# bharatlytics/faceRecognition_InfrenceEngine

Hardware: AMD Instinct MI355X
Metric: faces/sec end-to-end @1080p (higher is better)
Workload: dtype f16

## Files before the change

### facerecognition_infrenceengine_amd/_lib.py

```python
import ctypes as C
import struct
import os
import threading

_HERE = os.path.dirname(os.path.abspath(__file__))
LIB_PATH = os.path.join(_HERE, "csrc", "libfrhip.so")

_lock = threading.Lock()
_lib = None
ABI_VERSION = 106


class FrError(RuntimeError):
    pass


class ConvArgs(C.Structure):
    _fields_ = [("x", C.c_void_p), ("w", C.c_void_p), ("y", C.c_void_p),
                ("bias", C.c_void_p), ("slope", C.c_void_p), ("residual", C.c_void_p),
                ("out_f32_partial", C.c_void_p),
                ("B", C.c_int), ("H", C.c_int), ("W", C.c_int), ("Cin", C.c_int), ("Cout", C.c_int),
                ("KH", C.c_int), ("KW", C.c_int), ("stride", C.c_int), ("pad", C.c_int),
                ("Ho", C.c_int), ("Wo", C.c_int), ("bias_mode", C.c_int), ("splitk", C.c_int),
                ("x2", C.c_void_p), ("C2", C.c_int)]


class ConvStep(C.Structure):
    _fields_ = [("kind", C.c_int), ("args", ConvArgs)]


class ConvF8Args(C.Structure):
    _fields_ = [("x8", C.c_void_p), ("w8", C.c_void_p), ("y16", C.c_void_p), ("y8", C.c_void_p),
                ("oscale", C.c_void_p), ("bias", C.c_void_p), ("slope", C.c_void_p), ("residual", C.c_void_p),
                ("B", C.c_int), ("H", C.c_int), ("W", C.c_int), ("Cin", C.c_int), ("Cout", C.c_int),
                ("bias_mode", C.c_int), ("y8_mul", C.c_float), ("y8_sub", C.c_void_p)]


class RolePtr(C.c_void_p):
    role = None


class PnetLevel(C.Structure):
    _fields_ = [("x1", C.c_void_p), ("head", C.c_void_p), ("workspace", C.c_void_p), ("H1", C.c_int), ("W1", C.c_int),
                ("scale", C.c_float), ("boxes", C.c_void_p), ("scores", C.c_void_p), ("regs", C.c_void_p),
                ("counts", C.c_void_p), ("block_counts", C.c_void_p),
                ("x1s", C.c_void_p), ("hs", C.c_int), ("ws", C.c_int), ("f16", C.c_int)]


class FrameRef(C.Structure):
    _fields_ = [("data", C.c_void_p), ("H", C.c_int32), ("W", C.c_int32), ("nh", C.c_int32), ("nw", C.c_int32),
                ("reserved", C.c_int32 * 2)]


class Call(C.Structure):
    _fields_ = [("fn", C.c_int32), ("nargs", C.c_int32), ("a", C.c_uint64 * 22)]


_P, _I, _L, _F, _Z = C.c_void_p, C.c_int, C.c_int64, C.c_float, C.c_size_t
SEQ_FN = {"fr_dconv_mfma_f32": 1, "fr_pnet23_split_f16": 2, "fr_pnet_candidates": 3, "fr_sort_nms": 4, "fr_box_refine": 5,
          "fr_crop_conv1_f32": 6, "fr_stage_select": 7}

SIGNATURES = {
    "fr_version": (_I, []),
    "fr_last_error_string": (C.c_char_p, []),
    "fr_device_count": (_I, []),
    "fr_l2norm_rows_f32": (_I, [_P, _P, _I, _I, _P]),
    "fr_gallery_match_workspace": (_Z, [_I, _L]),
    "fr_gallery_match_f32": (_I, [_P, _P, _I, _L, _I, _L, _P, _P, _P, _Z, _P, _I, _P]),
    "fr_gallery_match_view_f32": (_I, [_P, _P, _P, _I, _L, _I, _P, _P, _P, _Z, _P]),
    "fr_gallery_topk_workspace": (_Z, [_I, _L, _I]),
    "fr_gallery_topk_f32": (_I, [_P, _P, _I, _L, _I, _I, _L, _P, _P, _P, _Z, _P, _I, _P]),
    "fr_gallery_topk_view_f32": (_I, [_P, _P, _P, _I, _L, _I, _I, _P, _P, _P, _Z, _P]),
    "fr_gallery_update_rows_f32": (_I, [_P, _P, _P, _I, _I, _I, _P]),
    "fr_gallery_match_f16_workspace": (_Z, [_I, _L]),
    "fr_gallery_match_f16": (_I, [_P, _P, _P, _I, _L, _I, _L, _P, _P, _P, _Z, _P, _I, _P]),
    "fr_gallery_match_f8_workspace": (_Z, [_I, _L]),
    "fr_gallery_match_f8": (_I, [_P, _P, _P, _I, _L, _I, _L, _P, _P, _P, _Z, _P, _I, _P]),
    "fr_gallery_update_rows_shadow": (_I, [_P, _P, _I, _P, _P, _I, _I, _I, _P]),
    "fr_gallery_match_view_f16_workspace": (_Z, [_I, _L]),
    "fr_gallery_match_view_f16": (_I, [_P, _P, _P, _P, _I, _L, _L, _I, _P, _P, _P, _Z, _P]),
    "fr_gallery_match_view_f8_workspace": (_Z, [_I, _L]),
    "fr_gallery_match_view_f8": (_I, [_P, _P, _P, _P, _I, _L, _L, _I, _P, _P, _P, _Z, _P]),
    "fr_gallery_topk_f16_workspace": (_Z, [_I, _L, _I]),
    "fr_gallery_topk_f16": (_I, [_P, _P, _P, _I, _L, _I, _I, _L, _P, _P, _P, _P, _P, _Z, _P, _I, _P]),
    "fr_gallery_topk_view_f16_workspace": (_Z, [_I, _L, _I]),
    "fr_gallery_topk_view_f16": (_I, [_P, _P, _P, _P, _I, _L, _L, _I, _I, _P, _P, _P, _P, _P, _Z, _P]),
    "fr_gallery_topk_view_masked_f32": (_I, [_P, _P, _P, _I, _L, _I, _I, _P, _P, _P, _Z, _P, _P]),
    "fr_gallery_match_grouped_workspace": (_Z, [_I, _L]),
    "fr_gallery_match_grouped_f32": (_I, [_P, _P, _P, _P, _P, _I, _I, _L, _L, _I, _P, _P, _P, _Z, _P, _I, _P]),
    "fr_gallery_topk_grouped_workspace": (_Z, [_I, _L, _I]),
    "fr_gallery_topk_grouped_f32": (_I, [_P, _P, _P, _P, _P, _I, _I, _L, _L, _I, _I, _P, _P, _P, _Z, _P, _I, _P]),
    "fr_gallery_gmax_update": (_I, [_P, _P, _L, _I, _P, _P]),
    "fr_f32_to_f8": (_I, [_P, _P, _L, _P]),
    "fr_f32_to_f16": (_I, [_P, _P, _L, _P]),
    "fr_match_decide": (_I, [_P, _P, _I, _F, _F, _P, _P]),
    "fr_match_pack_candidates": (_I, [_P, _P, _I, _P, _P]),
    "fr_match_reduce_shards": (_I, [_P, _I, _I, _I, _I, _P, _P, _P]),
    "fr_match_reduce_shards_topk": (_I, [_P, _I, _I, _I, _I, _I, _P, _P, _P]),
    "fr_exchange_pack_queries": (_I, [_P, _I, _I, _I, _P, _P]),
    "fr_exchange_counts": (_I, [_P, _I, _I, _I, _P, _P]),
    "fr_gallery_first_above_f32": (_I, [_P, _P, _I, _L, _I, _F, _I, _L, _P, _P, _P, _Z, _P]),
    "fr_cosine_matrix_f32": (_I, [_P, _P, _I, _I, _I, _P, _P]),
    "fr_mean_rows_f32": (_I, [_P, _I, _I, _P, _P]),
    "fr_unknown_assign_batch_f32": (_I, [_P, _P, _I, _I, _F, _P, _P, _P, _I, _I, _P, _P, _P, _P]),
    "fr_gallery_first_above_blocked_f32": (_I, [_P, _P, _P, _P, _I, _L, _I, _F, _I, _L, _P, _P, _P, _Z, _P]),
    "fr_enrol_batch_workspace": (_Z, [_I, _L]),
    "fr_enrol_batch_f32": (_I, [_P, _P, _I, _P, _P, _I, _P, _I, _I, _I, _P, _P, _L, _F, _F, _P, _P, _P, _P, _P, _P, _P, _P,
                                _Z, _P]),
    "fr_gallery_pairs_workspace": (_Z, [_L, _L]),
    "fr_gallery_pairs_above_f16": (_I, [_P, _P, _L, _I, _F, _I, _L, _I, _P, _P, _P, _P, _Z, _P]),
    "fr_conv_nhwc_f16": (_I, [C.POINTER(ConvArgs), _P]),
    "fr_conv_sequence": (_I, [C.POINTER(ConvStep), _I, _P]),
    "fr_conv_inblock_f16": (_I, [C.POINTER(ConvArgs), _P]),
    "fr_conv_nhwc_f8": (_I, [C.POINTER(ConvF8Args), _P]),
    "fr_quantize_f16_f8": (_I, [_P, _P, _L, _F, _P]),
    "fr_quantize_f16_f8_centred": (_I, [_P, _P, _L, _I, _P, _F, _P]),
    "fr_gptq_round_e4m3": (_I, [_P, _P, _P, _P, _I, _I, _P]),
    "fr_conv_stage14_weight_bytes": (_Z, [_I]),
    "fr_conv_stage14_pack": (_I, [_P, _P, _P]),
    "fr_conv_stage14_f16": (_I, [_P, _P, _P, _P, _I, _I, _P]),
    "fr_conv_walk64_weight_bytes": (_Z, [_I]),
    "fr_conv_walk64_pack": (_I, [_P, _P, _I, _P]),
    "fr_conv_walk64_f16": (_I, [_P, _P, _P, _P, _I, _P, _P, _I, _I, _I, _P]),
    "fr_conv_stage28_weight_bytes": (_Z, [_I]),
    "fr_conv_stage28_pack": (_I, [_P, _P, _P]),
    "fr_conv_stage28_f16": (_I, [_P, _P, _P, _P, _I, _I, _P]),
    "fr_conv_stage14_f8_weight_bytes": (_Z, [_I]),
    "fr_conv_stage14_f8_param_floats": (_Z, []),
    "fr_conv_stage14_f8_pack": (_I, [_P, _P, _P]),
    "fr_conv_stage14_f8": (_I, [_P, _P, _P, _P, _P, _I, _I, _P]),
    "fr_conv_splitk_epilogue": (_I, [_P, _I, _I, _I, _I, _I, _P, _I, _P, _P, _P, _P]),
    "fr_fc_reduce_l2norm": (_I, [_P, _I, _I, _I, _P, _P, _P, _P]),
    "fr_warp_affine_5pt": (_I, [_P, _I, _I, _I, _P, _P, _P, _I, _I, _P, _P, _P, _P]),
    "fr_warp_affine_5pt_slots": (_I, [_P, _I, _I, _I, _P, _P, _I, _I, _P, _P]),
    "fr_warp_affine_5pt_refs": (_I, [_P, _I, _P, _P, _P, _I, _I, _P, _P, _P, _P]),
    "fr_warp_affine_5pt_slots_refs": (_I, [_P, _I, _P, _P, _I, _I, _P, _P]),
    "fr_letterbox_u8": (_I, [_P, _I, _P, _I, _I, _P]),
    "fr_detections_unscale": (_I, [_P, _P, _P, _P, _I, _I, _P]),
    "fr_yuv420_to_bgr_u8": (_I, [_P, _P, _I, _I, _I, _I, _I, _I, _I, _I, _I, _I, _P]),
    "fr_yuv420_to_bgr_refs_u8": (_I, [_P, _P, _I, _I, _I, _I, _I, _I, _I, _I, _P]),
    "fr_frame_activity_u8": (_I, [_P, _I, _I, _I, _P, _I, _P, _P, _P, _I, _P, _P, _P, _I, _I, _I, _P]),
    "fr_frame_activity_refs_u8": (_I, [_P, _I, _P, _I, _P, _P, _P, _I, _P, _P, _P, _I, _I, _I, _P]),
    "fr_pyramid_resize_norm":(_I, [_P, _I, _I, _I, _I, _I, _P, _P]),
    "fr_dconv_f32": (_I, [_P, _P, _P, _P, _P, _I, _I, _I, _I, _I, _I, _I, _I, _I, _P, _P, _I, _P]),
    "fr_dconv_mfma_f32": (_I, [_I, _P, _P, _P, _P, _P, _I, _I, _I, _P, _P, _P, _I, _I, _P, _I, _P, _P]),
    "fr_crop_conv1_f32": (_I, [_I, _P, _I, _I, _I, _P, _P, _I, _P, _P, _P, _P, _P]),
    "fr_crop_conv1_split": (_I, [_I, _P, _I, _I, _I, _P, _P, _I, _P, _P, _P, _P, _I, _P]),
    "fr_crop_conv1_list_f32": (_I, [_I, _P, _I, _I, _I, _P, _I, _P, _P, _I, _P, _P, _P, _P, _P]),
    "fr_ro_conv2_split": (_I, [_I, _P, _P, _P, _P, _P, _I, _P, _I, _P, _P]),
    "fr_ro_gemm_weight_bytes": (_Z, [_I]),
    "fr_ro_gemm_pack": (_I, [_I, _P, _P, _P]),
    "fr_ro_gemm_split": (_I, [_I, _P, _P, _P, _P, _P, _I, _P, _I, _P]),
    "fr_ro_margin_list": (_I, [_P, _I, _P, _I, _I, _F, _F, _P, _P, _I, _P]),
    "fr_ro_scatter_rows": (_I, [_P, _P, _P, _I, _I, _P, _P]),
    "fr_pnet23_workspace_bytes": (_Z, [_I, _I, _I]),
    "fr_pnet23_split_f16": (_I, [_P, _P, _I, _I, _I, _P, _P, _P, _P, _P, _P, _P, _P, _P, _I, _F, _F, _P, _P, _Z, _P]),
    "fr_maxpool_f32": (_I, [_P, _P, _I, _I, _I, _I, _I, _I, _P]),
    "fr_pnet_conv1_band": (_I, [_I, _P, _I, _I, _I, _I, _I, _P, _P, _P, _P, _P, _P, _P, _I, _P]),
    "fr_pnet_band_tiles_count": (_Z, [_I, _I, _I]),
    "fr_pnet_band_tiles": (_I, [_P, _I, _I, _I, _P, _P, _P]),
    "fr_pnet_finish_levels": (_I, [C.POINTER(PnetLevel), _I, _I, _P, _P, _P, _P, _P, _P, _P, _P, _F, _I, _F, _P, _P]),
    "fr_pnet_pyramid_conv1": (_I, [_I, _P, _I, _I, _I, C.POINTER(PnetLevel), _I, _P, _P, _P, _P, _P, _I, _P]),
    "fr_pnet_pyramid_p23": (_I, [C.POINTER(PnetLevel), _I, _I, _P, _P, _P, _P, _P, _P, _P, _P, _I, _F, _F, _P]),
    "fr_pnet_pyramid_band_tiles": (_I, [C.POINTER(PnetLevel), _I, _I, _P, _P, _P]),
    "fr_pnet_candidates": (_I, [_P, _I, _I, _I, _F, _F, _I, _P, _P, _P, _P, _P, _P, _P, _F, _P]),
    "fr_sort_nms": (_I, [_P, _P, _P, _I, _P, _I, _I, _I, _I, _F, _I, _I, _P, _P, _P, _P, _I, _P]),
    "fr_box_refine": (_I, [_P, _P, _I, _P, _I, _I, _I, _P]),
    "fr_crop_resize_norm": (_I, [_P, _I, _I, _I, _P, _P, _I, _I, _P, _P]),
    "fr_stage_select": (_I, [_P, _P, _I, _P, _I, _I, _F, _P, _P, _P, _I, _P, _P, _P]),
    "fr_detect_sequence": (_I, [C.POINTER(Call), _I]),
    "fr_det_conv_weight_halves": (_Z, [_I, _I, _I]),
    "fr_det_conv_f16": (_I, [_P, _P, _P, _P, _P, _I, _I, _I, _I, _I, _I, _I, _I, _I, _I, _I, _I, _I, _I, _I, _P]),
    "fr_det_conv_act_f16": (_I, [_P, _P, _P, _P, _P, _P, _I, _I, _I, _I, _I, _I, _I, _I, _I, _I, _I, _I, _I, _I, _I, _P]),
    "fr_dw_conv_f16": (_I, [_P, _P, _P, _P, _P, _I, _I, _I, _I, _I, _I, _I, _I, _I, _I, _P]),
    "fr_det_input_f16": (_I, [_P, _P, _I, _I, _I, _P]),
    "fr_det_pool_f16": (_I, [_P, _P, _I, _I, _I, _I, _I, _I, _I, _I, _I, _I, _P]),
    "fr_det_upsample_add_f16": (_I, [_P, _P, _P, _I, _I, _I, _I, _I, _P]),
    "fr_scrfd_decode": (_I, [_P, _P, _P, _I, _I, _I, _I, _I, _I, _F, _P, _I, _P, _P, _P, _P, _P]),
}

_NOCHECK = ("fr_version", "fr_device_count")


def _slot(v, t):
    if t is _F:
        return struct.unpack("<I", struct.pack("<f", float(v)))[0]
    if t is _P:
        if v is None:
            return 0
        return int(v.value or 0) if isinstance(v, C.c_void_p) else int(v)
    return int(v) & 0xFFFFFFFFFFFFFFFF


class Lib:

    def __init__(self, cdll):
        self._c = cdll
        self._calls = {}
        self._rec = threading.local()
        for name, (res, args) in SIGNATURES.items():
            fn = getattr(cdll, name)
            fn.restype = res
            fn.argtypes = args
            if res is _I and name not in _NOCHECK:
                self._calls[name] = self._checked(name, fn)
            else:
                self._calls[name] = fn

    def _checked(self, name, fn):
        err = self._c.fr_last_error_string

        fid, types, rec = SEQ_FN.get(name), fn.argtypes, self._rec

        def call(*a):
            rc = fn(*a)
            if rc != 0:
                raise FrError(f"{name} failed ({rc}): {err().decode()}")
            if getattr(rec, "calls", None) is not None:
                rec.invalid = name
            return rc

        def call_rec(*a):
            rc = fn(*a)
            if rc != 0:
                raise FrError(f"{name} failed ({rc}): {err().decode()}")
            calls = getattr(rec, "calls", None)
            if calls is not None:
                calls.append((fid, [_slot(v, t) for v, t in zip(a, types)],
                              [(i, v.role) for i, v in enumerate(a) if isinstance(v, RolePtr)]))
            return rc
        return call_rec if fid is not None else call

    def start_recording(self):
        self._rec.calls, self._rec.invalid = [], None

    def note(self, fid, *slots):
        calls = getattr(self._rec, "calls", None)
        if calls is not None:
            calls.append((fid, [int(v.value or 0) if isinstance(v, C.c_void_p) else int(v) for v in slots], []))

    def stop_recording(self):
        calls, self._rec.calls = getattr(self._rec, "calls", None), None
        self._rec.last_invalid = getattr(self._rec, "invalid", None)
        self._rec.invalid = None
        return None if self._rec.last_invalid else calls

    def recording_invalid(self):
        return getattr(self._rec, "last_invalid", None)

    def __getattr__(self, name):
        try:
            return self.__dict__["_calls"][name]
        except KeyError:
            raise AttributeError(name)


def load():
    global _lib
    with _lock:
        if _lib is None:
            import torch
            if not os.path.exists(LIB_PATH):
                raise FrError(f"{LIB_PATH} not built: run `python -c 'import __graft_entry__ as g; g.build()'` "
                              f"or `make -C {os.path.dirname(LIB_PATH)}`; there is no CPU fallback")
            lib = Lib(C.CDLL(LIB_PATH))
            have = lib.fr_version()
            if have != ABI_VERSION:
                raise FrError(f"{LIB_PATH} implements ABI version {have}, this binding needs {ABI_VERSION}: rebuild it "
                              f"(`make -C {os.path.dirname(LIB_PATH)}`)")
            _lib = lib
        return _lib


def ptr(t, role=None):
    if t is None:
        return None
    if role is None:
        return C.c_void_p(t.data_ptr())
    p = RolePtr(t.data_ptr())
    p.role = role
    return p


def stream_ptr():
    import torch
    return C.c_void_p(torch.cuda.current_stream().cuda_stream)


def require_gpu():
    import torch
    if not torch.cuda.is_available():
        raise FrError("no HIP device visible: this engine has no CPU path")
```

### facerecognition_infrenceengine_amd/csrc/pnet_fused.hip

```cpp
#include "detect_math.h"

#define P23_RH 8
#define P23_RW 32
#define P23_X1W (P23_RW + 4)
#define P23_X1PX ((P23_RH + 4) * P23_X1W)
#define P23_X2W (P23_RW + 2)
#define P23_X2PX ((P23_RH + 2) * P23_X2W)
#define P23_X2T ((P23_X2PX + 15) / 16)
#define P23_NT 512
#define P23_X1PL (448 * 32)
#define P23_X2PL (P23_X2PX * 32)

struct P23Args {
    const float* x1;
    const unsigned char* x1s;
    unsigned x1s_bytes;
    const float* w2; const float* b2; const float* s2;
    const float* w3; const float* b3; const float* s3;
    const float* hw; const float* hb;
    float* head;
    float* dl;
    int all_heads;
    int* list; int* counts; int seg_cap;
    float logit_thr;
    float band_hi;
    int B, H1, W1, H3, W3, tiles_x, tiles_y, ntiles;
};

__device__ __forceinline__ void pnet23_body(const P23Args& a, const int vb, const int vgrid, char* lds) {
#if defined(__HIP_DEVICE_COMPILE__)
    char* x1t = lds;
    char* x2t = x1t + 2 * P23_X1PL;
    char* wf = x2t + 2 * P23_X2PL;
    float* cst = reinterpret_cast<float*>(wf + 30 * 1024);
    int* lcnt = reinterpret_cast<int*>(cst + 104);
    const int tid = threadIdx.x, lane = tid & 63, wave = tid >> 6;
    const int fr = lane & 15, fq = lane >> 4;

    for (int e = tid; e < 30 * 64; e += P23_NT) {
        const int l2 = e & 63, plane = (e >> 6) & 1, slot = e >> 7;
        const int r = l2 & 15, q = l2 >> 4;
        const bool c3 = slot >= 5;
        const int ct = c3 ? (slot - 5) / 5 : 0, ks = c3 ? (slot - 5) % 5 : slot;
        const float* w = (c3 ? a.w3 : a.w2) + ((size_t)(ct * 16 + r) * 10 + 2 * ks + (q >> 1)) * 16 + 8 * (q & 1);
        half8 o;
#pragma unroll
        for (int j = 0; j < 8; ++j) o[j] = split_f16_plane(w[j], plane);
        *reinterpret_cast<half8*>(wf + (size_t)e * 16) = o;
    }
    for (int e = tid; e < 16; e += P23_NT) { cst[e] = a.b2[e]; cst[16 + e] = a.s2[e] - 1.f; }
    for (int e = tid; e < 32; e += P23_NT) { cst[32 + e] = a.b3[e]; cst[64 + e] = a.s3[e] - 1.f; }
    for (int e = tid; e < 8; e += P23_NT) cst[96 + e] = e < 6 ? a.hb[e] : 0.f;
    if (tid == 0) *lcnt = 0;
    int* const seg = a.list + (size_t)vb * a.seg_cap;

    int off2[5], off3[5];
#pragma unroll
    for (int ks = 0; ks < 5; ++ks) {
        int t = 2 * ks + (fq >> 1);
        if (t > 8) t = 8;
        off2[ks] = ((t / 3) * P23_X1W + t % 3) * 32 + (fq & 1) * 16;
        off3[ks] = ((t / 3) * P23_X2W + t % 3) * 32 + (fq & 1) * 16;
    }

    __amdgpu_buffer_rsrc_t xrs = buffer_rsrc(a.x1s, a.x1s_bytes);
    int wy[4], wx[4], wc[4];
#pragma unroll
    for (int i = 0; i < 4; ++i) {
        const int j = wave + 8 * i, pl = j >= 14 ? 1 : 0;
        const int p = (j - 14 * pl) * 32 + (lane >> 1);
        wy[i] = p < P23_X1PX ? p / P23_X1W : 1 << 20; wx[i] = p % P23_X1W;
        wc[i] = pl * 32 + (lane & 1) * 16;
    }
    auto issue_window = [&](int tile) {
        const int per = a.tiles_x * a.tiles_y;
        const int n = tile / per, rem = tile - n * per;
        const int ty0 = (rem / a.tiles_x) * P23_RH, tx0 = (rem % a.tiles_x) * P23_RW;
#pragma unroll
        for (int i = 0; i < 4; ++i) {
            const int j = wave + 8 * i;
            if (j < 28) {
                const int gy = ty0 + wy[i], gx = tx0 + wx[i];
                const unsigned off = (gy < a.H1 && gx < a.W1) ? (unsigned)(((n * a.H1 + gy) * a.W1 + gx) * 64 + wc[i]) : 0x80000000u;
                __builtin_amdgcn_raw_ptr_buffer_load_lds(xrs, (lds_ptr_t)(x1t + (j >= 14 ? P23_X1PL + (j - 14) * 1024 : j * 1024)), 16, off, 0, 0, 0);
            }
        }
    };

    __syncthreads();
    half8 hwh, hwl;
#pragma unroll
    for (int j = 0; j < 8; ++j) {
        const int co = j < 4 ? 4 * fq + j : 16 + 4 * fq + (j - 4);
        const float w = fr < 6 ? a.hw[co * 6 + fr] : 0.f;
        split_f16(w, hwh, hwl, j);
    }
    issue_window(vb);
    for (int tile = vb; tile < a.ntiles; tile += vgrid) {
        const int per = a.tiles_x * a.tiles_y;
        const int n = tile / per, rem = tile - n * per;
        const int ty0 = (rem / a.tiles_x) * P23_RH, tx0 = (rem % a.tiles_x) * P23_RW;
        asm volatile("s_waitcnt vmcnt(0)" ::: "memory");
        __syncthreads();
        {
            const int t0 = wave < 6 ? wave * 3 : 18 + (wave - 6) * 2, nt = wave < 6 ? 3 : 2;
            int pb[3];
            float4v acc[3];
#pragma unroll
            for (int t = 0; t < 3; ++t) {
                int q = (t0 + t) * 16 + fr;
                if (q >= P23_X2PX) q = 0;
                pb[t] = ((q / P23_X2W) * P23_X1W + q % P23_X2W) * 32;
                acc[t] = float4v{0.f, 0.f, 0.f, 0.f};
            }
#pragma unroll
            for (int ks = 0; ks < 5; ++ks) {
                const half8 ahi = *reinterpret_cast<const half8*>(wf + ((ks * 2 + 0) * 64 + lane) * 16);
                const half8 alo = *reinterpret_cast<const half8*>(wf + ((ks * 2 + 1) * 64 + lane) * 16);
#pragma unroll
                for (int t = 0; t < 3; ++t) {
                    if (t < nt) {
                        const char* bp = x1t + (pb[t] + off2[ks]);
                        const half8 bhi = *reinterpret_cast<const half8*>(bp);
                        const half8 blo = *reinterpret_cast<const half8*>(bp + P23_X1PL);
                        acc[t] = __builtin_amdgcn_mfma_f32_16x16x32_f16(alo, bhi, acc[t], 0, 0, 0);
                        acc[t] = __builtin_amdgcn_mfma_f32_16x16x32_f16(ahi, blo, acc[t], 0, 0, 0);
                        acc[t] = __builtin_amdgcn_mfma_f32_16x16x32_f16(ahi, bhi, acc[t], 0, 0, 0);
                    }
                }
            }
            const float4v bb = *reinterpret_cast<const float4v*>(cst + 4 * fq), ss = *reinterpret_cast<const float4v*>(cst + 16 + 4 * fq);
#pragma unroll
            for (int t = 0; t < 3; ++t) {
                const int q = (t0 + t) * 16 + fr;
                if (t < nt && q < P23_X2PX) {
                    float4v v = acc[t] + bb;
#pragma unroll
                    for (int e = 0; e < 4; ++e) v[e] = __builtin_fmaf(fminf(v[e], 0.f), ss[e], v[e]);
                    half4 hi, lo;
#pragma unroll
                    for (int e = 0; e < 4; ++e) split_f16(v[e], hi, lo, e);
                    char* o = x2t + q * 32 + fq * 8;
                    *reinterpret_cast<half4*>(o) = hi;
                    *reinterpret_cast<half4*>(o + P23_X2PL) = lo;
                }
            }
        }
        __syncthreads();
        if (tile + vgrid < a.ntiles) issue_window(tile + vgrid);
        {
            int pb[2];
            float4v acc[2][2];
#pragma unroll
            for (int t = 0; t < 2; ++t) {
                const int q = (wave * 2 + t) * 16 + fr;
                pb[t] = ((q >> 5) * P23_X2W + (q & 31)) * 32;
                acc[t][0] = acc[t][1] = float4v{0.f, 0.f, 0.f, 0.f};
            }
#pragma unroll
            for (int ks = 0; ks < 5; ++ks) {
                half8 ahi[2], alo[2];
#pragma unroll
                for (int ct = 0; ct < 2; ++ct) {
                    ahi[ct] = *reinterpret_cast<const half8*>(wf + (((5 + ct * 5 + ks) * 2 + 0) * 64 + lane) * 16);
                    alo[ct] = *reinterpret_cast<const half8*>(wf + (((5 + ct * 5 + ks) * 2 + 1) * 64 + lane) * 16);
                }
#pragma unroll
                for (int t = 0; t < 2; ++t) {
                    const char* bp = x2t + (pb[t] + off3[ks]);
                    const half8 bhi = *reinterpret_cast<const half8*>(bp);
                    const half8 blo = *reinterpret_cast<const half8*>(bp + P23_X2PL);
#pragma unroll
                    for (int ct = 0; ct < 2; ++ct) {
                        acc[t][ct] = __builtin_amdgcn_mfma_f32_16x16x32_f16(alo[ct], bhi, acc[t][ct], 0, 0, 0);
                        acc[t][ct] = __builtin_amdgcn_mfma_f32_16x16x32_f16(ahi[ct], blo, acc[t][ct], 0, 0, 0);
                        acc[t][ct] = __builtin_amdgcn_mfma_f32_16x16x32_f16(ahi[ct], bhi, acc[t][ct], 0, 0, 0);
                    }
                }
            }
            const float4v b30 = *reinterpret_cast<const float4v*>(cst + 32 + 4 * fq), s30 = *reinterpret_cast<const float4v*>(cst + 64 + 4 * fq);
            const float4v b31 = *reinterpret_cast<const float4v*>(cst + 48 + 4 * fq), s31 = *reinterpret_cast<const float4v*>(cst + 80 + 4 * fq);
#pragma unroll
            for (int t = 0; t < 2; ++t) {
                float4v v0 = acc[t][0] + b30, v1 = acc[t][1] + b31;
                half8 bh, bl;
#pragma unroll
                for (int e = 0; e < 4; ++e) {
                    const float x0 = __builtin_fmaf(fminf(v0[e], 0.f), s30[e], v0[e]), x1 = __builtin_fmaf(fminf(v1[e], 0.f), s31[e], v1[e]);
                    const half_t h0 = (half_t)x0, h1 = (half_t)x1;
                    bh[e] = h0; bl[e] = (half_t)(x0 - (float)h0);
                    bh[4 + e] = h1; bl[4 + e] = (half_t)(x1 - (float)h1);
                }
                float4v d = {0.f, 0.f, 0.f, 0.f};
                d = __builtin_amdgcn_mfma_f32_16x16x32_f16(hwl, bh, d, 0, 0, 0);
                d = __builtin_amdgcn_mfma_f32_16x16x32_f16(hwh, bl, d, 0, 0, 0);
                d = __builtin_amdgcn_mfma_f32_16x16x32_f16(hwh, bh, d, 0, 0, 0);
                const int q = (wave * 2 + t) * 16 + fr;
                const int gy = ty0 + (q >> 5), gx = tx0 + (q & 31);
                const bool inb = fq < 2 && gy < a.H3 && gx < a.W3;
                const size_t cell = ((size_t)n * a.H3 + gy) * a.W3 + gx;
                const float4v hb4 = *reinterpret_cast<const float4v*>(cst + 96 + 4 * (fq & 1));
                const float o0 = d[0] + hb4[0], o1 = d[1] + hb4[1];
                const float dlv = __shfl(o1 - o0, fr, 64);
                const bool band = a.band_hi > a.logit_thr;
                const bool flag = inb && fq == 0 && (split_nonfinite(dlv) || (dlv >= a.logit_thr && (!band || dlv <= a.band_hi)));
                const unsigned long long fm = __ballot(flag);
                if (fm) {
                    int base = 0;
                    if (lane == (int)__builtin_ctzll(fm)) base = atomicAdd(lcnt, (int)__builtin_popcountll(fm));
                    base = __shfl(base, (int)__builtin_ctzll(fm), 64);
                    if (flag) seg[base + (int)__builtin_popcountll(fm & ((1ull << lane) - 1ull))] = (int)cell;
                }
                if (inb) {
                    if (fq == 0) a.dl[cell] = o1 - o0;
                    if (a.all_heads || (band && dlv >= a.logit_thr)) {
                        float* o = a.head + cell * 6 + 4 * fq;
                        *reinterpret_cast<float2*>(o) = make_float2(o0, o1);
                        if (fq == 0) *reinterpret_cast<float2*>(o + 2) = make_float2(d[2] + hb4[2], d[3] + hb4[3]);
                    }
                }
            }
        }
    }
    __syncthreads();
    if (tid == 0) a.counts[vb] = *lcnt;
#endif
}

__global__ __launch_bounds__(P23_NT, 4) void pnet23_split_f16(P23Args a) {
    extern __shared__ __attribute__((aligned(16))) char lds[];
    pnet23_body(a, (int)blockIdx.x, (int)gridDim.x, lds);
}

#define P23_MAXL 16
struct P23Levels {
    const unsigned char* x1s[P23_MAXL]; float* head[P23_MAXL]; float* dl[P23_MAXL];
    int H1[P23_MAXL], W1[P23_MAXL], seg_cap[P23_MAXL], first[P23_MAXL + 1];
    int nlevels;
};
__global__ __launch_bounds__(P23_NT, 4) void pnet23_split_levels(P23Args a, P23Levels t) {
    extern __shared__ __attribute__((aligned(16))) char lds[];
    int l = 0;
    while (l + 1 < t.nlevels && (int)blockIdx.x >= t.first[l + 1]) ++l;
    a.H1 = t.H1[l]; a.W1 = t.W1[l]; a.H3 = a.H1 - 4; a.W3 = a.W1 - 4;
    a.tiles_x = (a.W3 + P23_RW - 1) / P23_RW; a.tiles_y = (a.H3 + P23_RH - 1) / P23_RH;
    a.ntiles = a.B * a.tiles_x * a.tiles_y;
    a.x1s = t.x1s[l]; a.x1s_bytes = (unsigned)a.B * a.H1 * a.W1 * 64; a.head = t.head[l];
    a.dl = t.dl[l]; a.counts = reinterpret_cast<int*>(a.dl + (size_t)a.B * a.H3 * a.W3); a.list = a.counts + 512;
    a.seg_cap = t.seg_cap[l];
    pnet23_body(a, (int)blockIdx.x - t.first[l], t.first[l + 1] - t.first[l], lds);
}

#define PREF_WS 304
struct PRefArgs {
    const float* x1; const float* w2; const float* b2; const float* s2; const float* w3; const float* b3; const float* s3;
    const float* hw; const float* hb; float* head;
    const int* list; const int* counts; int seg_cap;
    int B, H1, W1, H3, W3;
    int* counter;
};

__device__ __forceinline__ void pnet_refine_body(const PRefArgs& a, const int block, float (*wins)[16 * PREF_WS], int (*cbase)[16]) {
#if defined(__HIP_DEVICE_COMPILE__)
    const int tid = threadIdx.x, lane = tid & 63, wave = tid >> 6;
    const int li = lane & 15, kq = lane >> 4;
    float* win = wins[wave];
    if (a.counts[block] <= wave * 16) return;
    float wa2[27], wa3[2][36], hwa[8];
#pragma unroll
    for (int s = 0; s < 27; ++s) wa2[s] = a.w2[(li * 10 + s / 3) * 16 + 4 * (s % 3) + kq];
#pragma unroll
    for (int i = 0; i < 2; ++i)
#pragma unroll
        for (int s = 0; s < 36; ++s) wa3[i][s] = a.w3[((16 * i + li) * 10 + s / 4) * 16 + 4 * (s % 4) + kq];
#pragma unroll
    for (int i = 0; i < 2; ++i)
#pragma unroll
        for (int e = 0; e < 4; ++e) hwa[i * 4 + e] = li < 6 ? a.hw[(16 * i + 4 * kq + e) * 6 + li] : 0.f;
    const float4v b2 = *reinterpret_cast<const float4v*>(a.b2 + 4 * kq), s2 = *reinterpret_cast<const float4v*>(a.s2 + 4 * kq);
    float4v b3[2], s3[2], hb4;
#pragma unroll
    for (int i = 0; i < 2; ++i) {
        b3[i] = *reinterpret_cast<const float4v*>(a.b3 + 16 * i + 4 * kq);
        s3[i] = *reinterpret_cast<const float4v*>(a.s3 + 16 * i + 4 * kq);
    }
#pragma unroll
    for (int r = 0; r < 4; ++r) hb4[r] = kq * 4 + r < 6 ? a.hb[kq * 4 + r] : 0.f;

    const int hw3 = a.H3 * a.W3;
    {
        const int* lst = a.list + (size_t)block * a.seg_cap;
        const int n_list = a.counts[block];
        if (a.counter && tid == 0 && n_list) atomicAdd(a.counter, n_list);
        for (int i0 = wave * 16; i0 < n_list; i0 += 64) {
            {
                const int c = lst[min(i0 + li, n_list - 1)];
                const int n = c / hw3, r = c - n * hw3, y = r / a.W3, x = r - y * a.W3;
                if (kq == 0) cbase[wave][li] = ((n * a.H1 + y) * a.W1 + x) * 12;
            }
            __builtin_amdgcn_wave_barrier();
            int l_ = lane;
            asm volatile("" : "+v"(l_));
            float4v pf[19];
#pragma unroll
            for (int it = 0; it < 19; ++it) {
                const int idx = min(it * 64 + l_, 1199);
                const int j = idx / 75, rem = idx - j * 75, row = rem / 15, c4 = rem - row * 15;
                pf[it] = *reinterpret_cast<const float4v*>(a.x1 + (size_t)(unsigned)cbase[wave][j] + (row * a.W1 * 12 + c4 * 4));
            }
#pragma unroll
            for (int it = 0; it < 19; ++it) {
                const int idx = it * 64 + l_;
                const int j = idx / 75, rem = idx - j * 75, row = rem / 15, c4 = rem - row * 15;
                if (it < 18 || l_ < 48) *reinterpret_cast<float4v*>(win + j * PREF_WS + row * 60 + c4 * 4) = pf[it];
            }
            __builtin_amdgcn_wave_barrier();
            const float* xb = win + li * PREF_WS + kq;
            float4v acc2[9];
#pragma unroll
            for (int p = 0; p < 9; ++p) acc2[p] = float4v{0.f, 0.f, 0.f, 0.f};
#pragma unroll
            for (int s = 0; s < 27; ++s) {
                const int tap = s / 3, c4 = s - tap * 3, ty = tap / 3, tx = tap - ty * 3;
#pragma unroll
                for (int p = 0; p < 9; ++p) {
                    const int py = p / 3, px = p - py * 3;
                    acc2[p] = __builtin_amdgcn_mfma_f32_16x16x4f32(wa2[s], xb[((py + ty) * 5 + px + tx) * 12 + 4 * c4], acc2[p], 0, 0, 0);
                }
            }
            __builtin_amdgcn_wave_barrier();
#pragma unroll
            for (int p = 0; p < 9; ++p) {
                float4v v = acc2[p] + b2;
#pragma unroll
                for (int e = 0; e < 4; ++e) v[e] = v[e] > 0.f ? v[e] : v[e] * s2[e];
                *reinterpret_cast<float4v*>(win + li * PREF_WS + p * 16 + 4 * kq) = v;
            }
            __builtin_amdgcn_wave_barrier();
            float4v acc3[2] = {float4v{0.f, 0.f, 0.f, 0.f}, float4v{0.f, 0.f, 0.f, 0.f}};
#pragma unroll
            for (int s = 0; s < 36; ++s) {
                const float bv = xb[(s / 4) * 16 + 4 * (s % 4)];
#pragma unroll
                for (int i = 0; i < 2; ++i) acc3[i] = __builtin_amdgcn_mfma_f32_16x16x4f32(wa3[i][s], bv, acc3[i], 0, 0, 0);
            }
            float4v hd = hb4;
#pragma unroll
            for (int i = 0; i < 2; ++i) {
                float4v v = acc3[i] + b3[i];
#pragma unroll
                for (int e = 0; e < 4; ++e) v[e] = v[e] > 0.f ? v[e] : v[e] * s3[i][e];
#pragma unroll
                for (int e = 0; e < 4; ++e) hd = __builtin_amdgcn_mfma_f32_16x16x4f32(hwa[i * 4 + e], v[e], hd, 0, 0, 0);
            }
            if (i0 + li < n_list && kq < 2) {
                float* o = a.head + (size_t)lst[i0 + li] * 6 + 4 * kq;
                *reinterpret_cast<float2*>(o) = make_float2(hd[0], hd[1]);
                if (kq == 0) *reinterpret_cast<float2*>(o + 2) = make_float2(hd[2], hd[3]);
            }
            __builtin_amdgcn_wave_barrier();
        }
    }
#endif
}

__global__ __launch_bounds__(256, 2) void pnet_refine_mfma(PRefArgs a) {
    __shared__ __attribute__((aligned(16))) float wins[4][16 * PREF_WS];
    __shared__ int cbase[4][16];
    pnet_refine_body(a, blockIdx.x, wins, cbase);
}

#define PREF_MAXL 16
struct PRefLevels {
    const float* x1[PREF_MAXL]; float* head[PREF_MAXL]; const int* list[PREF_MAXL]; const int* counts[PREF_MAXL];
    int seg_cap[PREF_MAXL], H1[PREF_MAXL], W1[PREF_MAXL], first[PREF_MAXL + 1];
    int nlevels;
};
__global__ __launch_bounds__(256, 2) void pnet_refine_levels(PRefArgs a, PRefLevels t) {
    __shared__ __attribute__((aligned(16))) float wins[4][16 * PREF_WS];
    __shared__ int cbase[4][16];
    int l = 0;
    while (l + 1 < t.nlevels && (int)blockIdx.x >= t.first[l + 1]) ++l;
    a.x1 = t.x1[l]; a.head = t.head[l]; a.list = t.list[l]; a.counts = t.counts[l]; a.seg_cap = t.seg_cap[l];
    a.H1 = t.H1[l]; a.W1 = t.W1[l]; a.H3 = t.H1[l] - 4; a.W3 = t.W1[l] - 4;
    pnet_refine_body(a, (int)blockIdx.x - t.first[l], wins, cbase);
}

static void p23_layout(int B, int H1, int W1, long long& ncell, long long& ntiles, int& grid, int& seg_cap) {
    const int H3 = H1 - 4, W3 = W1 - 4;
    ncell = (long long)B * H3 * W3;
    ntiles = (long long)B * ((W3 + P23_RW - 1) / P23_RW) * ((H3 + P23_RH - 1) / P23_RH);
    grid = (int)(ntiles < 512 ? ntiles : 512);
    seg_cap = (int)((ntiles + grid - 1) / (grid > 0 ? grid : 1)) * (P23_RH * P23_RW);
}
extern "C" size_t fr_pnet23_workspace_bytes(int B, int H1, int W1) {
    if (B <= 0 || H1 < 5 || W1 < 5) return 0;
    long long ncell, ntiles; int grid, seg_cap;
    p23_layout(B, H1, W1, ncell, ntiles, grid, seg_cap);
    return (size_t)ncell * 4 + 512 * 4 + (size_t)grid * seg_cap * 4;
}

extern "C" int fr_pnet23_split_f16(const float* x1, const void* x1s, int B, int H1, int W1, const float* w2, const float* b2,
                                   const float* s2, const float* w3, const float* b3, const float* s3, const float* hw,
                                   const float* hb, float* head, int all_heads, float refine_logit_thr, float refine_band_hi,
                                   int32_t* refined_count, void* workspace, size_t workspace_bytes, fr_stream_t stream) {
    FR_REQUIRE(x1 && x1s && w2 && b2 && s2 && w3 && b3 && s3 && hw && hb && head, "fr_pnet23_split_f16: null pointer");
    FR_REQUIRE((int64_t)B * H1 * W1 * 64 < (1ll << 31), "fr_pnet23_split_f16: the split conv1 map must stay below 2 GiB (got %lld bytes)", (long long)B * H1 * W1 * 64);
    FR_REQUIRE(B > 0 && H1 >= 5 && W1 >= 5, "fr_pnet23_split_f16: the conv1 map must be at least 5x5 (got %dx%d)", H1, W1);
    P23Args a;
    a.x1 = x1; a.x1s = (const unsigned char*)x1s; a.x1s_bytes = (unsigned)((int64_t)B * H1 * W1 * 64); a.w2 = w2; a.b2 = b2; a.s2 = s2; a.w3 = w3; a.b3 = b3; a.s3 = s3; a.hw = hw; a.hb = hb; a.head = head; a.all_heads = all_heads & 1;
    a.B = B; a.H1 = H1; a.W1 = W1; a.H3 = H1 - 4; a.W3 = W1 - 4;
    a.tiles_x = (a.W3 + P23_RW - 1) / P23_RW; a.tiles_y = (a.H3 + P23_RH - 1) / P23_RH;
    long long ncell, nt; int grid, seg_cap;
    p23_layout(B, H1, W1, ncell, nt, grid, seg_cap);
    FR_REQUIRE(nt < (1ll << 31) && ncell < (1ll << 31), "fr_pnet23_split_f16: too many tiles");
    const size_t need = fr_pnet23_workspace_bytes(B, H1, W1);
    FR_REQUIRE(workspace && workspace_bytes >= need, "fr_pnet23_split_f16: workspace needs %zu bytes (fr_pnet23_workspace_bytes)", need);
    a.dl = reinterpret_cast<float*>(workspace);
    a.counts = reinterpret_cast<int*>(a.dl + ncell);
    a.list = a.counts + 512;
    a.seg_cap = seg_cap;
    a.logit_thr = refine_logit_thr;
    a.band_hi = refine_band_hi;
    a.ntiles = (int)nt;
    constexpr size_t lds = (size_t)2 * P23_X1PL + (size_t)2 * P23_X2PL + 30 * 1024 + 108 * 4;
    static FrDevLatch latch;
    if (!fr_raise_lds(reinterpret_cast<const void*>(pnet23_split_f16), lds, latch)) { fr_set_error("fr_pnet23_split_f16: cannot raise dynamic LDS"); return FR_E_LAUNCH; }
    hipStream_t s = fr_stream(stream);
    pnet23_split_f16<<<grid, P23_NT, lds, s>>>(a);
    FR_CHECK_LAUNCH("pnet23_split_f16");
    if (all_heads & 2) return FR_OK;
    PRefArgs r;
    r.x1 = x1; r.w2 = w2; r.b2 = b2; r.s2 = s2; r.w3 = w3; r.b3 = b3; r.s3 = s3; r.hw = hw; r.hb = hb; r.head = head;
    r.list = a.list; r.counts = a.counts; r.seg_cap = seg_cap;
    r.B = B; r.H1 = H1; r.W1 = W1; r.H3 = a.H3; r.W3 = a.W3; r.counter = refined_count;
    pnet_refine_mfma<<<grid, 256, 0, s>>>(r);
    FR_CHECK_LAUNCH("pnet_refine_mfma");
    return FR_OK;
}

int fr_pnet_candidates_levels_launch(const fr_pnet_level* lv, int nlevels, int nframes, float thr, int cap, float dl_min, hipStream_t s);

extern "C" int fr_pnet_finish_levels(const fr_pnet_level* levels, int nlevels, int nframes, const float* w2, const float* b2,
                                     const float* s2, const float* w3, const float* b3, const float* s3, const float* hw,
                                     const float* hb, float thr, int cap, float dl_min, int32_t* refined_count, fr_stream_t stream) {
    FR_REQUIRE(levels && nlevels > 0 && nlevels <= PREF_MAXL && nframes > 0 && cap > 0, "fr_pnet_finish_levels: 1 .. %d levels", PREF_MAXL);
    FR_REQUIRE(w2 && b2 && s2 && w3 && b3 && s3 && hw && hb, "fr_pnet_finish_levels: null pointer");
    PRefLevels t;
    t.nlevels = nlevels;
    int total = 0;
    for (int l = 0; l < nlevels; ++l) {
        const fr_pnet_level& L = levels[l];
        FR_REQUIRE(L.x1 && L.head && L.workspace && L.boxes && L.scores && L.regs && L.counts && L.block_counts && L.H1 >= 5 && L.W1 >= 5 && L.scale > 0.f,
                   "fr_pnet_finish_levels: level %d: bad entry", l);
        long long ncell, nt; int grid, seg_cap;
        p23_layout(nframes, L.H1, L.W1, ncell, nt, grid, seg_cap);
        float* dl = reinterpret_cast<float*>(L.workspace);
        const int* counts = reinterpret_cast<const int*>(dl + ncell);
        t.x1[l] = L.x1; t.head[l] = L.head; t.counts[l] = counts; t.list[l] = counts + 512;
        t.seg_cap[l] = seg_cap; t.H1[l] = L.H1; t.W1[l] = L.W1;
        t.first[l] = total;
        total += grid;
    }
    t.first[nlevels] = total;
    PRefArgs r;
    r.x1 = nullptr; r.w2 = w2; r.b2 = b2; r.s2 = s2; r.w3 = w3; r.b3 = b3; r.s3 = s3; r.hw = hw; r.hb = hb; r.head = nullptr;
    r.list = nullptr; r.counts = nullptr; r.seg_cap = 0; r.B = nframes; r.H1 = r.W1 = r.H3 = r.W3 = 0; r.counter = refined_count;
    hipStream_t s = fr_stream(stream);
    pnet_refine_levels<<<total, 256, 0, s>>>(r, t);
    FR_CHECK_LAUNCH("pnet_refine_levels");
    return fr_pnet_candidates_levels_launch(levels, nlevels, nframes, thr, cap, dl_min, s);
}

__global__ __launch_bounds__(256) void pnet_band_tiles_kernel(const int* __restrict__ list, const int* __restrict__ counts, int seg_cap,
                                                             int H3, int W3, int regions_x, int regions_y, int32_t* __restrict__ tbuf,
                                                             int32_t* __restrict__ tiles) {
    const int n_list = counts[blockIdx.x];
    const int* lst = list + (size_t)blockIdx.x * seg_cap;
    const int hw3 = H3 * W3;
    for (int i = threadIdx.x; i < n_list; i += 256) {
        const int c = lst[i];
        const int n = c / hw3, r = c - n * hw3, y = r / W3, x = r - y * W3;
        const int ry0 = (2 * y) >> 4, ry1 = min((2 * y + 9) >> 4, regions_y - 1);
        const int rx0 = (2 * x) >> 6, rx1 = min((2 * x + 9) >> 6, regions_x - 1);
        for (int ry = ry0; ry <= ry1; ++ry)
            for (int rx = rx0; rx <= rx1; ++rx) {
                const int t = (n * regions_y + ry) * regions_x + rx;
                const unsigned bit = 1u << (t & 31);
                const unsigned old = atomicOr(reinterpret_cast<unsigned*>(tbuf) + 1 + (t >> 5), bit);
                if (!(old & bit)) tiles[atomicAdd(tbuf, 1)] = t;
            }
    }
}

extern "C" size_t fr_pnet_band_tiles_count(int B, int H1, int W1) {
    if (B <= 0 || H1 < 5 || W1 < 5) return 0;
    return (size_t)B * ((H1 + 7) / 8) * ((W1 + 31) / 32);
}

extern "C" int fr_pnet_band_tiles(const void* workspace, int B, int H1, int W1, int32_t* tbuf, int32_t* tiles, fr_stream_t stream) {
    FR_REQUIRE(workspace && tbuf && tiles && B > 0 && H1 >= 5 && W1 >= 5, "fr_pnet_band_tiles: bad argument");
    long long ncell, nt; int grid, seg_cap;
    p23_layout(B, H1, W1, ncell, nt, grid, seg_cap);
    const float* dl = reinterpret_cast<const float*>(workspace);
    const int* counts = reinterpret_cast<const int*>(dl + ncell);
    const int regions_y = (H1 + 7) / 8, regions_x = (W1 + 31) / 32;
    const size_t ntile = (size_t)B * regions_y * regions_x;
    hipStream_t s = fr_stream(stream);
    if (hipMemsetAsync(tbuf, 0, (1 + (ntile + 31) / 32) * sizeof(int32_t), s) != hipSuccess) { fr_set_error("fr_pnet_band_tiles: memset failed"); return FR_E_LAUNCH; }
    pnet_band_tiles_kernel<<<grid, 256, 0, s>>>(counts + 512, counts, seg_cap, H1 - 4, W1 - 4, regions_x, regions_y, tbuf, tiles);
    FR_CHECK_LAUNCH("pnet_band_tiles_kernel");
    return FR_OK;
}

extern "C" int fr_pnet_pyramid_p23(const fr_pnet_level* levels, int nlevels, int nframes, const float* w2, const float* b2,
                                   const float* s2, const float* w3, const float* b3, const float* s3, const float* hw,
                                   const float* hb, int all_heads, float refine_logit_thr, float refine_band_hi, fr_stream_t stream) {
    FR_REQUIRE(levels && nlevels > 0 && nlevels <= P23_MAXL && nframes > 0, "fr_pnet_pyramid_p23: 1 .. %d levels", P23_MAXL);
    FR_REQUIRE(w2 && b2 && s2 && w3 && b3 && s3 && hw && hb, "fr_pnet_pyramid_p23: null pointer");
    P23Levels t;
    t.nlevels = nlevels;
    long long total = 0;
    for (int l = 0; l < nlevels; ++l) {
        const fr_pnet_level& L = levels[l];
        FR_REQUIRE(L.x1s && L.head && L.workspace && L.H1 >= 5 && L.W1 >= 5, "fr_pnet_pyramid_p23: level %d: bad entry", l);
        FR_REQUIRE((int64_t)nframes * L.H1 * L.W1 * 64 < (1ll << 31), "fr_pnet_pyramid_p23: level %d: the split conv1 map must stay below 2 GiB", l);
        long long ncell, nt; int grid, seg_cap;
        p23_layout(nframes, L.H1, L.W1, ncell, nt, grid, seg_cap);
        t.x1s[l] = reinterpret_cast<const unsigned char*>(L.x1s); t.head[l] = L.head; t.dl[l] = reinterpret_cast<float*>(L.workspace);
        t.H1[l] = L.H1; t.W1[l] = L.W1; t.seg_cap[l] = seg_cap;
        t.first[l] = (int)total;
        total += grid;
    }
    t.first[nlevels] = (int)total;
    P23Args a{};
    a.w2 = w2; a.b2 = b2; a.s2 = s2; a.w3 = w3; a.b3 = b3; a.s3 = s3; a.hw = hw; a.hb = hb; a.all_heads = all_heads & 1;
    a.logit_thr = refine_logit_thr; a.band_hi = refine_band_hi; a.B = nframes;
    constexpr size_t lds = (size_t)2 * P23_X1PL + (size_t)2 * P23_X2PL + 30 * 1024 + 108 * 4;
    static FrDevLatch latch;
    if (!fr_raise_lds(reinterpret_cast<const void*>(pnet23_split_levels), lds, latch)) { fr_set_error("fr_pnet_pyramid_p23: cannot raise dynamic LDS"); return FR_E_LAUNCH; }
    pnet23_split_levels<<<(unsigned)total, P23_NT, lds, fr_stream(stream)>>>(a, t);
    FR_CHECK_LAUNCH("pnet23_split_levels");
    return FR_OK;
}

struct PBandLevels {
    const int* counts[PREF_MAXL];
    int seg_cap[PREF_MAXL], H1[PREF_MAXL], W1[PREF_MAXL], word0[PREF_MAXL], level[PREF_MAXL], first[PREF_MAXL + 1];
    int nlevels;
};
__global__ __launch_bounds__(256) void pnet_band_tiles_levels(PBandLevels t, int32_t* __restrict__ tbuf, int32_t* __restrict__ tiles, int cap) {
    int l = 0;
    while (l + 1 < t.nlevels && (int)blockIdx.x >= t.first[l + 1]) ++l;
    const int b = (int)blockIdx.x - t.first[l];
    const int n_list = t.counts[l][b];
    const int* lst = t.counts[l] + 512 + (size_t)b * t.seg_cap[l];
    const int H3 = t.H1[l] - 4, W3 = t.W1[l] - 4, hw3 = H3 * W3;
    const int regions_y = (t.H1[l] + 7) / 8, regions_x = (t.W1[l] + 31) / 32;
    unsigned* bitmap = reinterpret_cast<unsigned*>(tbuf) + 1 + t.word0[l];
    for (int i = threadIdx.x; i < n_list; i += 256) {
        const int c = lst[i];
        const int n = c / hw3, r = c - n * hw3, y = r / W3, x = r - y * W3;
        const int ry0 = (2 * y) >> 4, ry1 = min((2 * y + 9) >> 4, regions_y - 1);
        const int rx0 = (2 * x) >> 6, rx1 = min((2 * x + 9) >> 6, regions_x - 1);
        for (int ry = ry0; ry <= ry1; ++ry)
            for (int rx = rx0; rx <= rx1; ++rx) {
                const int tl = (n * regions_y + ry) * regions_x + rx;
                const unsigned bit = 1u << (tl & 31);
                const unsigned old = atomicOr(bitmap + (tl >> 5), bit);
                if (!(old & bit)) {
                    const int at = atomicAdd(tbuf, 1);
                    if (at < cap) tiles[at] = (t.level[l] << 27) | tl;
                }
            }
    }
}

extern "C" int fr_pnet_pyramid_band_tiles(const fr_pnet_level* levels, int nlevels, int nframes, int32_t* tbuf, int32_t* tiles,
                                          fr_stream_t stream) {
    FR_REQUIRE(levels && nlevels > 0 && nlevels <= PREF_MAXL && nframes > 0 && tbuf && tiles, "fr_pnet_pyramid_band_tiles: bad argument");
    PBandLevels t;
    t.nlevels = 0;
    long long blocks = 0, words = 0, cap = 0;
    for (int l = 0; l < nlevels; ++l) {
        const fr_pnet_level& L = levels[l];
        if (!L.f16) continue;
        FR_REQUIRE(L.workspace && L.H1 >= 5 && L.W1 >= 5, "fr_pnet_pyramid_band_tiles: level %d: bad entry", l);
        long long ncell, nt; int grid, seg_cap;
        p23_layout(nframes, L.H1, L.W1, ncell, nt, grid, seg_cap);
        const long long ntile = (long long)fr_pnet_band_tiles_count(nframes, L.H1, L.W1);
        FR_REQUIRE(ntile < (1ll << 27), "fr_pnet_pyramid_band_tiles: level %d: too many tiles", l);
        const int k = t.nlevels++;
        t.counts[k] = reinterpret_cast<const int*>(reinterpret_cast<const float*>(L.workspace) + ncell);
        t.seg_cap[k] = seg_cap; t.H1[k] = L.H1; t.W1[k] = L.W1; t.word0[k] = (int)words; t.level[k] = l;
        t.first[k] = (int)blocks;
        blocks += grid; words += (ntile + 31) / 32; cap += ntile;
    }
    FR_REQUIRE(t.nlevels > 0 && cap < (1ll << 31), "fr_pnet_pyramid_band_tiles: no level in the f16 form");
    t.first[t.nlevels] = (int)blocks;
    hipStream_t s = fr_stream(stream);
    if (hipMemsetAsync(tbuf, 0, (size_t)(1 + words) * sizeof(int32_t), s) != hipSuccess) { fr_set_error("fr_pnet_pyramid_band_tiles: memset failed"); return FR_E_LAUNCH; }
    pnet_band_tiles_levels<<<(unsigned)blocks, 256, 0, s>>>(t, tbuf, tiles, (int)cap);
    FR_CHECK_LAUNCH("pnet_band_tiles_levels");
    return FR_OK;
}
```

### facerecognition_infrenceengine_amd/mtcnn.py

```python
import contextlib
import ctypes
import functools
import logging
import math
import threading
from types import SimpleNamespace
from typing import NamedTuple

import torch

from . import _lib


def pyramid_scales(h, w, minsize=20, factor=0.709):
    m = 12.0 / minsize
    minl = min(h, w) * m
    scales, k = [], 0
    while minl >= 12:
        scales.append(m * factor ** k)
        minl *= factor
        k += 1
    return scales


def _pool_out(n, k, s):
    o = -(-(n - k) // s) + 1
    if (o - 1) * s >= n:
        o -= 1
    return o


MFMA_LAYERS = {0: (3, 12, 3, 3, 1), 1: (12, 16, 3, 3, 1), 2: (16, 32, 3, 3, 2),
               10: (4, 28, 3, 3, 2), 11: (28, 48, 3, 3, 3), 12: (48, 64, 2, 2, 4), 13: (64, 128, 3, 3, 4),
               14: (128, 6, 1, 1, 1),
               20: (4, 32, 3, 3, 1), 21: (32, 64, 3, 3, 2), 22: (64, 64, 3, 3, 4), 23: (64, 128, 2, 2, 4),
               24: (128, 256, 3, 3, 4), 25: (256, 16, 1, 1, 1)}


class _MConv:

    def __init__(self, layer, w, b, slope, device, head=None):
        cin, cout, kh, kw, ntb = MFMA_LAYERS[layer]
        rcout, rcin = w.shape[0], w.shape[1]
        assert tuple(w.shape[2:]) == (kh, kw) and rcout <= cout and rcin <= cin, (layer, tuple(w.shape))
        wfull = torch.zeros((cout, cin, kh, kw), dtype=torch.float32)
        wfull[:rcout, :rcin] = w
        w = wfull
        bfull = torch.zeros(cout); bfull[:rcout] = b; b = bfull
        if slope is not None:
            sfull = torch.zeros(cout); sfull[:rcout] = slope; slope = sfull
        self.layer, self.cin, self.cout, self.kh, self.kw = layer, cin, cout, kh, kw
        cinp = -(-cin // 4) * 4
        cp = ntb * 16 + (16 if ntb % 2 == 0 else 0)
        gsz = ntb * 16
        ngroups = -(-cout // gsz)
        wp = torch.zeros((ngroups, kh * kw, cinp, cp), dtype=torch.float32)
        wt = w.permute(2, 3, 1, 0).reshape(kh * kw, cin, cout)
        for g in range(ngroups):
            n = min(gsz, cout - g * gsz)
            wp[g, :, :cin, :n] = wt[:, :, g * gsz:g * gsz + n]
        self.w = wp.contiguous().to(device)
        bp = torch.zeros(ngroups * gsz); bp[:cout] = b
        self.b = bp.to(device)
        self.slope = None
        if slope is not None:
            sp = torch.zeros(ngroups * gsz); sp[:cout] = slope
            self.slope = sp.to(device)
        self.head_w = self.head_b = None
        self.nhead = 0
        if head is not None:
            self.head_w = head[0].t().contiguous().to(torch.float32).to(device)
            self.head_b = head[1].to(torch.float32).contiguous().to(device)
            self.nhead = head[0].shape[0]
        self.pool = {0: 2, 10: 3, 11: 3, 20: 3, 21: 3, 22: 2}.get(layer, 0)

    def out_hw(self, h, w):
        hc, wc = h - self.kh + 1, w - self.kw + 1
        return (_pool_out(hc, self.pool, 2), _pool_out(wc, self.pool, 2)) if self.pool else (hc, wc)


_CHAINS = {"pnet": (("conv1", ("conv2",)), ("conv2", ("conv3",)), ("conv3", ("conv4_1", "conv4_2"))),
           "rnet": (("conv1", ("conv2",)), ("conv2", ("conv3",)), ("conv3", ("dense4",)), ("dense4", ("dense5_1", "dense5_2"))),
           "onet": (("conv1", ("conv2",)), ("conv2", ("conv3",)), ("conv3", ("conv4",)), ("conv4", ("dense5",)),
                    ("dense5", ("dense6_1", "dense6_2", "dense6_3")))}


def canonical_scale(state, net, dead_zone=2):
    st = dict(state)
    for name, readers in _CHAINS[net]:
        w = st[name + ".weight"]
        rms = float(w.double().pow(2).mean().sqrt())
        if rms == 0.0:
            continue
        e = math.log2(math.sqrt(2.0 / w[0].numel()) / rms)
        k = int(round(e)) if abs(e) > dead_zone else 0
        if k:
            st[name + ".weight"] = w * 2.0 ** k
            st[name + ".bias"] = st[name + ".bias"] * 2.0 ** k
            for n in readers:
                st[n + ".weight"] = st[n + ".weight"] * 2.0 ** -k
    return st


def _dense_as_conv(w, k, c):
    o = w.shape[0]
    return w.reshape(o, k, k, c).permute(0, 3, 2, 1).contiguous()


class DetectSettings:
    SINGLE_FRAME_LEVEL_STREAMS = 4
    one_stream = False
    level_streams = 2
    phase_marks = None
    solo_max_frames = 7
    pnet_band = True
    split_pconv1 = True
    split_pconv1_min_px = 10000
    pyramid_launch = True
    refined_cells = None
    use_sequence = True
    fused_crop = True
    split_ro = True

    def __init__(self, minsize=20, factor=0.709, fused_pnet=True, batch_min_pixels=None):
        self.minsize, self.factor = minsize, factor
        self.fused_pnet = bool(fused_pnet)
        self.batch_min_pixels = 22_000_000 if batch_min_pixels is None else int(batch_min_pixels)
        self.single_frame_level_streams = self.SINGLE_FRAME_LEVEL_STREAMS


class DetectPlan(NamedTuple):
    N: int
    scales: tuple
    geo: tuple
    batch: bool
    few: bool
    band: bool
    fused: tuple
    f16: tuple
    pyramid: bool
    solo: bool
    nside: int
    cache: bool
    recorder: bool
    split: bool
    chunks: tuple


def _is_batch(cfg, N, H, W):
    return N * H * W >= cfg.batch_min_pixels


def _level_geo(H, W, scale):
    hs, ws = int(math.ceil(H * scale)), int(math.ceil(W * scale))
    return hs, ws, _pool_out(hs - 2, 2, 2), _pool_out(ws - 2, 2, 2)


def _frames32(h, w):
    return (2 ** 31 - 1) // (h * w * 64)


def _f16_conv1(cfg, band, h, w):
    return bool(band and cfg.split_pconv1 and h * w >= cfg.split_pconv1_min_px)


def detect_plan(N, H, W, cfg, trace=False, level_streams=None, out=False, capturing=False):
    return _plan(N, H, W, tuple([getattr(cfg, k) for k in _PLAN_READS]), cfg.phase_marks is None and cfg.refined_cells is None,
                 trace, level_streams, out, capturing)


_PLAN_READS = ("minsize", "factor", "fused_pnet", "batch_min_pixels", "solo_max_frames", "pnet_band", "split_pconv1", "split_pconv1_min_px",
               "pyramid_launch", "one_stream", "level_streams", "single_frame_level_streams", "split_ro", "fused_crop", "use_sequence")


@functools.lru_cache(maxsize=256)
def _plan(N, H, W, settings, recordable, trace, level_streams, out, capturing):
    cfg = SimpleNamespace(**dict(zip(_PLAN_READS, settings)))
    scales = tuple(pyramid_scales(H, W, cfg.minsize, cfg.factor))
    geo = tuple(_level_geo(H, W, s) for s in scales)
    batch = _is_batch(cfg, N, H, W)
    few = N <= cfg.solo_max_frames and not batch
    fusable = bool(cfg.fused_pnet) and not trace
    chunks, per = (), N
    if fusable and not out and N > 1 and geo and 1 <= _frames32(*geo[0][2:]) < N:
        per = -(-N // -(-N // _frames32(*geo[0][2:])))
        chunks = tuple((n0, min(N, n0 + per)) for n0 in range(0, N, per))
    band = bool(cfg.pnet_band and batch and not trace)
    fused = tuple(bool(cfg.fused_pnet) and per <= _frames32(h, w) for _, _, h, w in geo)
    f16 = tuple(fu and _f16_conv1(cfg, band, h, w) for fu, (_, _, h, w) in zip(fused, geo))
    pyramid = bool(cfg.pyramid_launch and batch and fusable and all(fused))
    nside = max(1, min(2, level_streams if level_streams is not None else cfg.level_streams))
    own = few and level_streams is None
    if own and capturing and cfg.single_frame_level_streams > 0:
        nside = min(cfg.single_frame_level_streams, max(1, len(scales) - 1))
    eager = bool(trace or cfg.one_stream or (own and not capturing))
    cache = bool(eager and few and not trace and not out and not capturing)
    recorder = bool(cache and recordable and cfg.use_sequence and cfg.fused_pnet and cfg.fused_crop and not cfg.one_stream)
    split = bool(cfg.split_ro and cfg.fused_crop and batch and not trace)
    return DetectPlan(N, scales, geo, batch, few, band, fused, f16, pyramid, eager or pyramid, nside, cache, recorder, split, chunks)


_RO = (SimpleNamespace(name="rnet", cap_in="cap_p", cap_out="cap_r", crop=24, map1=(11, 28), map2=(4, 48), w1="_rc1", w2="_rc2",
                       layers=("r1", "r2", "r3", "r4", "r5"), nhead=6, naux=4, refine=1),
       SimpleNamespace(name="onet", cap_in="cap_r", cap_out="cap_o", crop=48, map1=(23, 32), map2=(10, 64), w1="_oc1", w2="_oc2",
                       layers=("o1", "o2", "o3", "o4", "o5", "o6"), nhead=16, naux=14, refine=2))


class MTCNNHIP(DetectSettings):
    def __init__(self, pstate, rstate, ostate, device="cuda:0", minsize=20, factor=0.709,
                 thresholds=(0.6, 0.7, 0.7), cap_scale=2048, keep_scale=256, cap_p=512, cap_r=64, cap_o=16,
                 fused_pnet=True, batch_min_pixels=None, canonical=True):
        _lib.require_gpu()
        DetectSettings.__init__(self, minsize, factor, fused_pnet, batch_min_pixels)
        self.lib = _lib.load()
        self.device = torch.device(device)
        self.thresholds = tuple(float(t) for t in thresholds)
        self.cap_scale, self.keep_scale, self.cap_p, self.cap_r, self.cap_o = cap_scale, keep_scale, cap_p, cap_r, cap_o
        assert cap_scale <= 4096 and cap_p <= 1024 and cap_r <= 1024 and cap_o <= 1024
        self._sides = {}
        self._tls = threading.local()
        self._unfused_logged = False
        d = self.device
        p, r, o = ({k: v.detach().float().cpu() for k, v in s.items()} for s in (pstate, rstate, ostate))
        if canonical:
            p, r, o = (canonical_scale(s, n) for s, n in ((p, "pnet"), (r, "rnet"), (o, "onet")))
        self.p1 = _MConv(0, p["conv1.weight"], p["conv1.bias"], p["prelu1.weight"], d)
        self.p2 = _MConv(1, p["conv2.weight"], p["conv2.bias"], p["prelu2.weight"], d)
        hw = torch.cat([p["conv4_1.weight"].reshape(2, 32), p["conv4_2.weight"].reshape(4, 32)])
        hb = torch.cat([p["conv4_1.bias"], p["conv4_2.bias"]])
        self.p3 = _MConv(2, p["conv3.weight"], p["conv3.bias"], p["prelu3.weight"], d, head=(hw, hb))
        w2p = torch.zeros((16, 10, 16)); w2p[:, :9, :10] = p["conv2.weight"].permute(0, 2, 3, 1).reshape(16, 9, 10)
        w3p = torch.zeros((32, 10, 16)); w3p[:, :9, :16] = p["conv3.weight"].permute(0, 2, 3, 1).reshape(32, 9, 16)
        self._p23 = tuple(t.to(torch.float32).contiguous().to(d) for t in (
            w2p, p["conv2.bias"], p["prelu2.weight"], w3p, p["conv3.bias"], p["prelu3.weight"], hw.t().contiguous(), hb))
        self.refine_margin = 2e-3
        self.level_tensors = None
        self.p23_all_heads = False
        self._rc1 = tuple(t.to(torch.float32).contiguous().to(d) for t in (
            r["conv1.weight"].permute(2, 3, 1, 0).reshape(27, 28), r["conv1.bias"], r["prelu1.weight"]))
        self._oc1 = tuple(t.to(torch.float32).contiguous().to(d) for t in (
            o["conv1.weight"].permute(2, 3, 1, 0).reshape(27, 32), o["conv1.bias"], o["prelu1.weight"]))
        self.split_conv1 = True
        self.ro_margin = 1e-3
        self.ro_list_cap = (1024, 256)
        def c2w(w):
            o, c = w.shape[0], w.shape[1]
            wp = torch.zeros((o, 9, 32))
            wp[:, :, :c] = w.permute(0, 2, 3, 1).reshape(o, 9, c)
            return wp
        self._rc2 = tuple(t.to(torch.float32).contiguous().to(d) for t in (c2w(r["conv2.weight"]), r["conv2.bias"], r["prelu2.weight"]))
        self._oc2 = tuple(t.to(torch.float32).contiguous().to(d) for t in (c2w(o["conv2.weight"]), o["conv2.bias"], o["prelu2.weight"]))
        self.r1 = _MConv(10, r["conv1.weight"], r["conv1.bias"], r["prelu1.weight"], d)
        self.r2 = _MConv(11, r["conv2.weight"], r["conv2.bias"], r["prelu2.weight"], d)
        self.r3 = _MConv(12, r["conv3.weight"], r["conv3.bias"], r["prelu3.weight"], d)
        self.r4 = _MConv(13, _dense_as_conv(r["dense4.weight"], 3, 64), r["dense4.bias"], r["prelu4.weight"], d)
        self.r5 = _MConv(14, torch.cat([r["dense5_1.weight"], r["dense5_2.weight"]]).reshape(6, 128, 1, 1),
                         torch.cat([r["dense5_1.bias"], r["dense5_2.bias"]]), None, d)
        self.o1 = _MConv(20, o["conv1.weight"], o["conv1.bias"], o["prelu1.weight"], d)
        self.o2 = _MConv(21, o["conv2.weight"], o["conv2.bias"], o["prelu2.weight"], d)
        self.o3 = _MConv(22, o["conv3.weight"], o["conv3.bias"], o["prelu3.weight"], d)
        self.o4 = _MConv(23, o["conv4.weight"], o["conv4.bias"], o["prelu4.weight"], d)
        self.o5 = _MConv(24, _dense_as_conv(o["dense5.weight"], 3, 128), o["dense5.bias"], o["prelu5.weight"], d)
        self._gemm = {}
        for lid, wconv, b, sl in ((12, r["conv3.weight"], r["conv3.bias"], r["prelu3.weight"]),
                                  (13, _dense_as_conv(r["dense4.weight"], 3, 64), r["dense4.bias"], r["prelu4.weight"]),
                                  (22, o["conv3.weight"], o["conv3.bias"], o["prelu3.weight"]),
                                  (23, o["conv4.weight"], o["conv4.bias"], o["prelu4.weight"]),
                                  (24, _dense_as_conv(o["dense5.weight"], 3, 128), o["dense5.bias"], o["prelu5.weight"])):
            wk = wconv.permute(0, 2, 3, 1).reshape(wconv.shape[0], -1).to(torch.float32).contiguous().to(d)
            packed = torch.empty(self.lib.fr_ro_gemm_weight_bytes(lid), dtype=torch.uint8, device=d)
            with torch.cuda.device(d):
                self.lib.fr_ro_gemm_pack(lid, _lib.ptr(wk), _lib.ptr(packed), _lib.stream_ptr())
                torch.cuda.synchronize(d)
            self._gemm[lid] = (packed, b.to(torch.float32).contiguous().to(d), sl.to(torch.float32).contiguous().to(d))
        self.o6 = _MConv(25, torch.cat([o["dense6_1.weight"], o["dense6_2.weight"], o["dense6_3.weight"]]).reshape(16, 256, 1, 1),
                         torch.cat([o["dense6_1.bias"], o["dense6_2.bias"], o["dense6_3.bias"]]), None, d)

    def set_exact(self, on=True):
        self.pnet_band = self.split_ro = not on
        return self

    @property
    def _dl(self):
        return getattr(self._tls, "dl", (None, 0.0))

    @property
    def _s(self):
        return self._tls.s

    @_s.setter
    def _s(self, v):
        self._tls.s = v

    def _new(self, shape, dtype):
        c = getattr(self._tls, "cache", None)
        if c is None:
            return torch.empty(shape, dtype=dtype, device=self.device)
        lst, i = c
        c[1] = i + 1
        if i < len(lst) and lst[i].shape == tuple(shape) and lst[i].dtype == dtype:
            return lst[i]
        t = torch.empty(shape, dtype=dtype, device=self.device)
        self._tls.cache_grew = True
        if i < len(lst):
            lst[i] = t
        else:
            lst.append(t)
        return t

    def _f32(self, *shape):
        return self._new(shape, torch.float32)

    def _i32(self, *shape):
        return self._new(shape, torch.int32)

    def _fptr(self, frames):
        return _lib.ptr(frames, role="frame")

    def _dconv(self, x, c, B, H, W, frames=None, counts=None, cap=0, y_split=None, y=None):
        ho, wo = c.out_hw(H, W)
        if y is None:
            y = self._f32(B, ho, wo, c.nhead if c.nhead else c.cout)
        fh, fw = (frames.shape[1], frames.shape[2]) if frames is not None else (0, 0)
        self.lib.fr_dconv_mfma_f32(c.layer, _lib.ptr(x), _lib.ptr(c.w), _lib.ptr(c.b), _lib.ptr(c.slope), _lib.ptr(y),
                                   B, H, W, _lib.ptr(c.head_w), _lib.ptr(c.head_b), self._fptr(frames), fh, fw,
                                   _lib.ptr(counts), cap, _lib.ptr(y_split), self._s)
        return y, ho, wo

    def _gemm_split(self, lid, x, B, shape, counts, cap):
        w, b, sl = self._gemm[lid]
        y = self._f32(B, *shape)
        self.lib.fr_ro_gemm_split(lid, _lib.ptr(x), _lib.ptr(w), _lib.ptr(b), _lib.ptr(sl), _lib.ptr(y), B, _lib.ptr(counts), cap, self._s)
        return y

    def _nms(self, boxes, scores, aux, naux, counts, L, nseg, seg_cap, seg_major, thr, mode, keep, out=None, results=False):
        if out is None:
            bo, so, co = self._f32(L, keep, 4), self._f32(L, keep), self._i32(L)
            ao = self._f32(L, keep, max(naux, 1))
        else:
            bo, so, ao, co = out
        po = [_lib.ptr(t, role="out%d" % i if results else None) for i, t in enumerate((bo, so, ao, co))]
        self.lib.fr_sort_nms(_lib.ptr(boxes), _lib.ptr(scores), _lib.ptr(aux), naux, _lib.ptr(counts), L, nseg, seg_cap,
                             seg_major, thr, mode, keep, *po, keep, self._s)
        return bo, so, ao, co

    def _band_logits(self, band=True):
        lt = math.log(self.thresholds[0] / (1.0 - self.thresholds[0]))
        return lt - self.refine_margin, lt + self.refine_margin if band else float("-inf")

    def _level_buffers(self, N, scale, geo, band, f16, cand):
        hs, ws, h, w = geo
        path = getattr(self._tls, "path", None)
        if path is not None:
            path["fused_levels"] += 1
            path["band_levels"] += int(band)
            if f16:
                path["pconv1_mfma_levels"].append((h, w))
        xs = self._new((N, h, w, 64), torch.uint8)
        x = self._f32(N, h, w, 12)
        head = self._f32(N, h - 4, w - 4, 6)
        wsp = self._new((self.lib.fr_pnet23_workspace_bytes(N, h, w) // 4,), torch.float32)
        bc = self._i32(N * (-(-(h - 4) * (w - 4) // 256)))
        entry = None
        if cand is not None:
            entry = _lib.PnetLevel(x.data_ptr(), head.data_ptr(), wsp.data_ptr(), h, w, float(scale), *[t.data_ptr() for t in cand],
                                   bc.data_ptr(), xs.data_ptr(), hs, ws, int(f16))
        return dict(h=h, w=w, f16=f16, x=x, xs=xs, head=head, wsp=wsp, bc=bc), entry

    def _level(self, frames, scale, geo, fused, band, f16, trace, cand):
        N, H, W, _ = frames.shape
        hs, ws, h, w = geo
        lib, p1 = self.lib, self.p1
        if not fused:
            if self.fused_pnet and not self._unfused_logged:
                self._unfused_logged = True
                logging.getLogger(__name__).warning("MTCNNHIP: a %d x %d pyramid level of %d frame(s) exceeds the fused P-Net's 32-bit map "
                                                    "offsets; it runs layer by layer (f32)", hs, ws, N)
            if getattr(self._tls, "path", None) is not None:
                self._tls.path["unfused_levels"] += 1
            x, h, w = self._dconv(None, p1, N, hs, ws, frames=frames)
            x, h, w = self._dconv(x, self.p2, N, h, w)
            head, h, w = self._dconv(x, self.p3, N, h, w)
            return head, h, w, self._i32(N * (-(-h * w // 256))), None, 0.0, None
        lo, hi = self._band_logits(band)
        t, entry = self._level_buffers(N, scale, geo, band, f16, cand[3:] if f16 else None)
        x, xs, head, wsp = t["x"], t["xs"], t["head"], t["wsp"]
        p1w, p23 = (_lib.ptr(p1.w), _lib.ptr(p1.b), _lib.ptr(p1.slope)), [_lib.ptr(v) for v in self._p23]
        if f16:
            lib.fr_pnet_conv1_band(0, self._fptr(frames), N, H, W, hs, ws, *p1w, None, _lib.ptr(xs), None, None, 0, self._s)
        else:
            self._dconv(None, p1, N, hs, ws, frames=frames, y_split=xs, y=x)
        lib.fr_pnet23_split_f16(_lib.ptr(x), _lib.ptr(xs), N, h, w, *p23, _lib.ptr(head),
                                (1 if (self.p23_all_heads or trace is not None) else 0) | (2 if f16 else 0), lo, hi,
                                _lib.ptr(self.refined_cells), _lib.ptr(wsp), wsp.numel() * 4, self._s)
        keep = None
        if f16:
            nt = lib.fr_pnet_band_tiles_count(N, h, w)
            tbuf, tiles = self._i32(1 + (nt + 31) // 32), self._i32(nt)
            lib.fr_pnet_band_tiles(_lib.ptr(wsp), N, h, w, _lib.ptr(tbuf), _lib.ptr(tiles), self._s)
            lib.fr_pnet_conv1_band(1, self._fptr(frames), N, H, W, hs, ws, *p1w, _lib.ptr(x), None, _lib.ptr(tiles), _lib.ptr(tbuf), nt, self._s)
            lib.fr_pnet_finish_levels((_lib.PnetLevel * 1)(entry), 1, N, *p23, cand[1], cand[2], lo, _lib.ptr(self.refined_cells), self._s)
            t.update(tbuf=tbuf, tiles=tiles)
            keep = (x, xs, head, wsp, tbuf, tiles, t["bc"])
        if self.level_tensors is not None:
            self.level_tensors.append(t)
        return head, h - 4, w - 4, t["bc"], wsp, lo, keep

    def pnet_level(self, frames, scale, trace=None, cand=None):
        N, H, W, _ = frames.shape
        geo = _level_geo(H, W, scale)
        fused = bool(self.fused_pnet) and N <= _frames32(*geo[2:])
        band = bool(self.pnet_band and _is_batch(self, N, H, W) and trace is None)
        f16 = fused and cand is not None and _f16_conv1(self, band, *geo[2:])
        head, hc, wc, _, dl, dl_min, keep = self._level(frames, scale, geo, fused, band, f16, trace, cand)
        self._tls.dl, self._tls.level_done, self._tls.keep = (dl, dl_min), keep is not None, keep
        return head, hc, wc

    def _pnet_pyramid(self, frames, plan, cand):
        N, H, W, _ = frames.shape
        lib, p1, nlev = self.lib, self.p1, len(plan.scales)
        lo, hi = self._band_logits(plan.band)
        lv = (_lib.PnetLevel * nlev)()
        keep, ntile, words = [], 0, 0
        for li, (s, geo, f16) in enumerate(zip(plan.scales, plan.geo, plan.f16)):
            t, lv[li] = self._level_buffers(N, s, geo, plan.band, f16, [c[li] for c in cand])
            keep.append(t)
            if f16:
                nt = lib.fr_pnet_band_tiles_count(N, t["h"], t["w"])
                ntile, words = ntile + nt, words + (nt + 31) // 32
        p1w, p23 = (_lib.ptr(p1.w), _lib.ptr(p1.b), _lib.ptr(p1.slope)), [_lib.ptr(t) for t in self._p23]
        lib.fr_pnet_pyramid_conv1(0, self._fptr(frames), N, H, W, lv, nlev, *p1w, None, None, 0, self._s)
        lib.fr_pnet_pyramid_p23(lv, nlev, N, *p23, 1 if self.p23_all_heads else 0, lo, hi, self._s)
        if ntile:
            tbuf, tiles = self._i32(1 + words), self._i32(ntile)
            lib.fr_pnet_pyramid_band_tiles(lv, nlev, N, _lib.ptr(tbuf), _lib.ptr(tiles), self._s)
            lib.fr_pnet_pyramid_conv1(1, self._fptr(frames), N, H, W, lv, nlev, *p1w, _lib.ptr(tiles), _lib.ptr(tbuf), ntile, self._s)
            keep[0].update(tbuf=tbuf, tiles=tiles)
        lib.fr_pnet_finish_levels(lv, nlev, N, *p23, self.thresholds[0], self.cap_scale, lo, _lib.ptr(self.refined_cells), self._s)
        if self.level_tensors is not None:
            self.level_tensors.extend(keep)

    @contextlib.contextmanager
    def _forked(self, main, n, events=None):
        note = self.lib.note
        sides = self._sides.setdefault(main.cuda_stream, [])
        while len(sides) < n:
            sides.append(torch.cuda.Stream(device=self.device))
        sides = sides[:n]
        if events is None:
            for side in sides:
                side.wait_stream(main)
        else:
            events[0].record(main)
            note(8, events[0].cuda_event, main.cuda_stream)
            for side in sides:
                side.wait_event(events[0])
                note(9, side.cuda_stream, events[0].cuda_event)
        yield sides
        if events is None:
            for side in sides:
                main.wait_stream(side)
        else:
            for side, ev in zip(sides, events[1:]):
                ev.record(side)
                note(8, ev.cuda_event, side.cuda_stream)
                main.wait_event(ev)
                note(9, main.cuda_stream, ev.cuda_event)
        self._s = ctypes.c_void_p(main.cuda_stream)

    def _pnet_levels(self, frames, plan, trace, cand):
        N, lib, t0, cs = plan.N, self.lib, self.thresholds[0], self.cap_scale
        events = (self._tls.rec or {}).get("events")
        forked = events is not None or not plan.solo
        main, keep = torch.cuda.current_stream(), []
        with (self._forked(main, len(events) - 1 if events else plan.nside, events) if forked else contextlib.nullcontext()) as sides:
            for li, s in enumerate(plan.scales):
                stream = sides[(li - 1) % len(sides)] if forked and li else main
                with (contextlib.nullcontext() if plan.solo else torch.cuda.stream(stream)):
                    if forked:
                        self._s = ctypes.c_void_p(stream.cuda_stream)
                    lcand = [c[li] for c in cand]
                    head, hc, wc, bc, dl, dl_min, done = self._level(
                        frames, s, plan.geo[li], plan.fused[li], plan.band, plan.f16[li], trace,
                        (float(s), t0, cs, *lcand) if plan.batch and trace is None else None)
                    prob = self._f32(N, hc, wc) if trace is not None else None
                    if done is not None:
                        keep.append(done)
                    else:
                        lib.fr_pnet_candidates(_lib.ptr(head), N, hc, wc, float(s), t0, cs, *[_lib.ptr(c) for c in lcand], _lib.ptr(bc),
                                               _lib.ptr(prob), _lib.ptr(dl), dl_min, self._s)
                    if trace is not None:
                        trace.setdefault("pnet_head", []).append(head)
                        trace.setdefault("pnet_prob", []).append(prob)
        for grp in keep:
            for t in grp:
                t.record_stream(main)

    def _stage1(self, frames, plan, trace):
        N, nlev, cs, ksz = plan.N, len(plan.scales), self.cap_scale, self.keep_scale
        lb, ls, lr, lc = self._f32(nlev, N, cs, 4), self._f32(nlev, N, cs), self._f32(nlev, N, cs, 4), self._i32(nlev, N)
        kb, ks, ka, kc = self._f32(nlev, N, ksz, 4), self._f32(nlev, N, ksz), self._f32(nlev, N, ksz, 4), self._i32(nlev, N)
        if self.level_tensors is not None:
            del self.level_tensors[:]
        if plan.pyramid:
            self._pnet_pyramid(frames, plan, (lb, ls, lr, lc))
        else:
            self._pnet_levels(frames, plan, trace, (lb, ls, lr, lc))
        self._mark("pnet")
        if self.level_tensors is not None:
            self.level_tensors.append(dict(cand=(lb, ls, lr, lc)))
        self._nms(lb, ls, lr, 4, lc, nlev * N, 1, cs, 0, 0.5, 0, ksz, out=(kb, ks, ka, kc))
        b1, s1, a1, c1 = self._nms(kb, ks, ka, 4, kc, N, nlev, ksz, 1, 0.7, 0, self.cap_p)
        self.lib.fr_box_refine(_lib.ptr(b1), _lib.ptr(a1), 4, _lib.ptr(c1), N, self.cap_p, 0, self._s)
        self._mark("stage1_nms")
        if trace is not None:
            trace.update(stage1_boxes=b1, stage1_scores=s1, stage1_counts=c1)
        return b1, s1, a1, c1

    def crop_conv1(self, net, frames, boxes, counts, cap):
        N, H, W, _ = frames.shape
        t = _RO[net]
        w, b, s = getattr(self, t.w1)
        y = self._f32(N * cap, t.map1[0], t.map1[0], t.map1[1])
        self.lib.fr_crop_conv1_f32(net, self._fptr(frames), N, H, W, _lib.ptr(boxes), _lib.ptr(counts), cap, _lib.ptr(w),
                                   _lib.ptr(b), _lib.ptr(s), _lib.ptr(y), self._s)
        return y

    def crop_conv12_split(self, net, frames, boxes, counts, cap):
        N, H, W, _ = frames.shape
        t = _RO[net]
        (w1, b1, s1), (w2, b2, s2) = getattr(self, t.w1), getattr(self, t.w2)
        xs = self._new((N * cap, t.map1[0] ** 2, 128), torch.uint8)
        self.lib.fr_crop_conv1_split(net, self._fptr(frames), N, H, W, _lib.ptr(boxes), _lib.ptr(counts), cap, _lib.ptr(w1),
                                     _lib.ptr(b1), _lib.ptr(s1), _lib.ptr(xs), 1 if self.split_conv1 else 0, self._s)
        y = self._f32(N * cap, t.map2[0], t.map2[0], t.map2[1])
        lc = self._i32(1)
        self.lib.fr_ro_conv2_split(net, _lib.ptr(xs), _lib.ptr(w2), _lib.ptr(b2), _lib.ptr(s2), _lib.ptr(y), N * cap,
                                   _lib.ptr(counts), cap, _lib.ptr(lc), self._s)
        return y, lc

    def exact_pass(self, net, frames, boxes, counts, cap, head, thr, lc):
        N, H, W, _ = frames.shape
        t = _RO[net]
        w1, b1, s1 = getattr(self, t.w1)
        lcap, nh = self.ro_list_cap[net], head.shape[1]
        lst = self._i32(lcap)
        self.lib.fr_ro_margin_list(_lib.ptr(head), nh, _lib.ptr(counts), N, cap, math.log(thr / (1.0 - thr)), self.ro_margin,
                                   _lib.ptr(lst), _lib.ptr(lc), lcap, self._s)
        x1 = self._f32(lcap, t.map1[0], t.map1[0], t.map1[1])
        self.lib.fr_crop_conv1_list_f32(net, self._fptr(frames), N, H, W, _lib.ptr(boxes), cap, _lib.ptr(lst), _lib.ptr(lc), lcap,
                                        _lib.ptr(w1), _lib.ptr(b1), _lib.ptr(s1), _lib.ptr(x1), self._s)
        exact = getattr(self, t.name)(None, lcap, lc, lcap, x1=x1)
        self.lib.fr_ro_scatter_rows(_lib.ptr(exact), _lib.ptr(lst), _lib.ptr(lc), lcap, nh, _lib.ptr(head), self._s)
        self._tls.__dict__.setdefault("ro_lists", {})[net] = lc
        self._tls.path["exact_lists"].append((net, lcap))
        self._tls.exact_counters.append(lc)

    @property
    def _ro_lists(self):
        return getattr(self._tls, "ro_lists", {})

    def exact_lists(self):
        path = getattr(self._tls, "path", None)
        if not path:
            return []
        torch.cuda.synchronize(self.device)
        return [{"net": _RO[net].name, "count": int(lc[0]), "cap": cap}
                for (net, cap), lc in zip(path["exact_lists"], self._tls.exact_counters)]

    def exact_list_overflow(self):
        return sorted({e["net"] for e in self.exact_lists() if e["count"] > e["cap"]}, key=("rnet", "onet").index)

    def _net(self, t, x, B, counts, cap, x1, x2):
        k = dict(counts=counts, cap=cap)
        layers = [getattr(self, n) for n in t.layers]
        if x2 is not None:
            x, h, w = x2, t.map2[0], t.map2[0]
        else:
            x, h, w = (x1, t.map1[0], t.map1[0]) if x1 is not None else self._dconv(x, layers[0], B, t.crop, t.crop, **k)
            x, h, w = self._dconv(x, layers[1], B, h, w, **k)
        for c in layers[2:-1]:
            if x2 is not None:
                h, w = c.out_hw(h, w)
                x = self._gemm_split(c.layer, x, B, (h, w, c.cout), counts, cap)
            else:
                x, h, w = self._dconv(x, c, B, h, w, **k)
        x, _, _ = self._dconv(x, layers[-1], B, 1, 1, **k)
        return x.reshape(B, t.nhead)

    def rnet(self, x, B, counts=None, cap=0, x1=None, x2=None):
        return self._net(_RO[0], x, B, counts, cap, x1, x2)

    def onet(self, x, B, counts=None, cap=0, x1=None, x2=None):
        return self._net(_RO[1], x, B, counts, cap, x1, x2)

    def _refine_stage(self, net, frames, boxes, counts, plan, trace, out=None):
        t = _RO[net]
        N, H, W, _ = frames.shape
        lib, run, thr, crops = self.lib, getattr(self, t.name), self.thresholds[1 + net], None
        cap, cap_out = getattr(self, t.cap_in), getattr(self, t.cap_out)
        if plan.split:
            y, lc = self.crop_conv12_split(net, frames, boxes, counts, cap)
            head = run(None, N * cap, counts, cap, x2=y)
            self.exact_pass(net, frames, boxes, counts, cap, head, thr, lc)
        elif self.fused_crop and trace is None:
            head = run(None, N * cap, counts, cap, x1=self.crop_conv1(net, frames, boxes, counts, cap))
        else:
            crops = self._f32(N * cap, t.crop, t.crop, 4)
            lib.fr_crop_resize_norm(self._fptr(frames), N, H, W, _lib.ptr(boxes), _lib.ptr(counts), cap, t.crop, _lib.ptr(crops), self._s)
            head = run(crops, N * cap, counts, cap)
        sb, ss, sa, sc = self._f32(N, cap, 4), self._f32(N, cap), self._f32(N, cap, t.naux), self._i32(N)
        prob = self._f32(N, cap) if trace is not None else None
        lib.fr_stage_select(_lib.ptr(boxes), _lib.ptr(head), t.nhead, _lib.ptr(counts), N, cap, thr, _lib.ptr(sb), _lib.ptr(ss),
                            _lib.ptr(sa), t.naux, _lib.ptr(sc), _lib.ptr(prob), self._s)
        if net == 0:
            res = self._nms(sb, ss, sa, t.naux, sc, N, 1, cap, 0, 0.7, 0, cap_out)
            lib.fr_box_refine(_lib.ptr(res[0]), _lib.ptr(res[2]), t.naux, _lib.ptr(res[3]), N, cap_out, t.refine, self._s)
        else:
            lib.fr_box_refine(_lib.ptr(sb), _lib.ptr(sa), t.naux, _lib.ptr(sc), N, cap, t.refine, self._s)
            self._tls.cache = None
            res = self._nms(sb, ss, sa, t.naux, sc, N, 1, cap, 0, 0.7, 1, cap_out, out=out, results=True)
        self._mark("stage%d" % (2 + net))
        if trace is not None:
            trace.update({t.name + "_head": head, t.name + "_prob": prob})
            if net == 0:
                trace.update(rnet_crops=crops, stage2_boxes=res[0], stage2_scores=res[1], stage2_counts=res[3])
        return res

    def _mark(self, name):
        if self.phase_marks is not None:
            e = torch.cuda.Event(enable_timing=True)
            e.record()
            self.phase_marks.append((name, e))

    def _begin(self, frames, plan):
        tls = self._tls
        tls.rec = None
        if not plan.cache:
            return None
        caches, seqs = tls.__dict__.setdefault("caches", {}), tls.__dict__.setdefault("seqs", {})
        key = (*frames.shape[:3], torch.cuda.current_stream().cuda_stream)
        if key not in caches and len(caches) >= 4:
            old_key = next(iter(caches))
            caches.pop(old_key); seqs.pop(old_key, None)
        known = key in caches
        tls.cache = [caches.setdefault(key, []), 0]
        cfg = (self.fused_pnet, self.fused_crop, self.p23_all_heads, self.thresholds, self.refine_margin,
               self.cap_scale, self.keep_scale, self.cap_p, self.cap_r, self.cap_o, self.minsize, self.factor)
        seq = seqs.get(key)
        if seq is not None and (not plan.recorder or seq["cfg"] != cfg):
            seqs.pop(key)
            seq = None
        if seq is not None:
            tls.cache = None
            return seq
        tls.rec = {"key": key, "cfg": cfg, "events": None}
        if plan.recorder and known:
            self.lib.start_recording()
            tls.rec["events"] = [torch.cuda.Event() for _ in range(1 + min(4, max(1, len(plan.scales) - 1)))]

    def _end(self, frames, outs):
        tls = self._tls
        rec, tls.rec = tls.rec, None
        if rec is None:
            return
        if rec["events"] is not None:
            calls = self.lib.stop_recording()
            if calls and not tls.cache_grew:
                seq = self._make_sequence(calls, frames, outs, rec["cfg"])
                if seq is not None:
                    seq["events"] = rec["events"]
                    tls.seqs[rec["key"]] = seq
        if tls.cache_grew:
            tls.seqs.pop(rec["key"], None)

    def detect_batch(self, frames, trace=None, level_streams=None, _out=None):
        assert frames.dtype == torch.uint8 and frames.dim() == 4 and frames.shape[3] == 3 and frames.is_contiguous()
        N, H, W, _ = frames.shape
        with torch.cuda.device(self.device):
            plan = detect_plan(N, H, W, self, trace is not None, level_streams, _out is not None, torch.cuda.is_current_stream_capturing())
            if _out is None:
                self._tls.path = {"frames": N, "batch": plan.batch, "chunks": max(1, len(plan.chunks)), "fused_levels": 0, "band_levels": 0,
                                  "pconv1_mfma_levels": [], "unfused_levels": 0, "split_ro": False, "exact_lists": []}
                self._tls.exact_counters = []
            if plan.chunks:
                out = tuple(torch.empty(sh, dtype=dt, device=self.device) for sh, dt in (
                    ((N, self.cap_o, 4), torch.float32), ((N, self.cap_o), torch.float32), ((N, self.cap_o, 14), torch.float32), ((N,), torch.int32)))
                for n0, n1 in plan.chunks:
                    self.detect_batch(frames[n0:n1], None, level_streams, _out=tuple(t[n0:n1] for t in out))
                return out[0], out[1], out[2][..., 4:14].unflatten(-1, (5, 2)), out[3]
            self._s = _lib.stream_ptr()
            self._tls.cache, self._tls.cache_grew = None, False
            self.lib.stop_recording()
            self._mark("start")
            if not plan.scales:
                z = torch.zeros((N, self.cap_o, 14), dtype=torch.float32, device=self.device)
                return (z[..., :4].contiguous(), z[..., 0].contiguous(), z[..., 4:14].unflatten(-1, (5, 2)),
                        torch.zeros(N, dtype=torch.int32, device=self.device))
            assert len(plan.scales) * self.keep_scale <= 4096, "too many pyramid levels for the merged NMS list"
            seq = self._begin(frames, plan)
            if seq is not None:
                return self._replay(seq, frames)
            b1, _, _, c1 = self._stage1(frames, plan, trace)
            self._tls.path["split_ro"] = plan.split
            b2, _, _, c2 = self._refine_stage(0, frames, b1, c1, plan, trace)
            b3, s3, a3, c3 = self._refine_stage(1, frames, b2, c2, plan, trace, out=_out)
            self._end(frames, (b3, s3, a3, c3))
            return b3, s3, a3[..., 4:14].unflatten(-1, (5, 2)), c3

    def _make_sequence(self, calls, frames, outs, cfg):
        log = logging.getLogger(__name__)
        arr = (_lib.Call * len(calls))()
        want = {"frame": frames.data_ptr(), **{"out%d" % i: t.data_ptr() for i, t in enumerate(outs)}}
        fpos, opos = [], [[] for _ in outs]
        for k, (fid, slots, roles) in enumerate(calls):
            arr[k].fn, arr[k].nargs = fid, len(slots)
            for i, v in enumerate(slots):
                arr[k].a[i] = v
            tagged = dict(roles)
            for i, role in roles:
                if slots[i] != want[role]:
                    log.warning("MTCNNHIP: recorded call %d: slot %d carries the role '%s' but holds another tensor; call list refused", k, i, role)
                    return None
                (fpos if role == "frame" else opos[int(role[3:])]).append((k, i))
            if fid < 8:
                for i, v in enumerate(slots):
                    if i not in tagged and v in want.values():
                        log.warning("MTCNNHIP: recorded call %d: slot %d holds a patched tensor without its role; call list refused", k, i)
                        return None
        if not fpos or not all(opos):
            log.warning("MTCNNHIP: the recorded call list does not mention the frame and every result tensor; refused")
            return None
        return {"arr": arr, "n": len(calls), "fpos": fpos, "opos": opos, "cfg": cfg,
                "meta": [(tuple(t.shape), t.dtype) for t in outs]}

    def _replay(self, seq, frames):
        arr = seq["arr"]
        outs = [torch.empty(shape, dtype=dtype, device=self.device) for shape, dtype in seq["meta"]]
        fptr = frames.data_ptr()
        for k, i in seq["fpos"]:
            arr[k].a[i] = fptr
        for t, pos in zip(outs, seq["opos"]):
            p = t.data_ptr()
            for k, i in pos:
                arr[k].a[i] = p
        self.lib.fr_detect_sequence(arr, seq["n"])
        b3, s3, a3, c3 = outs
        return b3, s3, a3[..., 4:14].unflatten(-1, (5, 2)), c3
```

### include/frhip.h

```cpp
#ifndef FRHIP_H
#define FRHIP_H
#include <stddef.h>
#include <stdint.h>
#ifdef __cplusplus
extern "C" {
#endif

#define FR_OK 0
#define FR_E_INVALID (-1)
#define FR_E_LAUNCH (-2)
#define FR_E_NODEVICE (-3)

typedef void* fr_stream_t;

#define FR_ABI_VERSION 106
int fr_version(void);
const char* fr_last_error_string(void);
int fr_device_count(void);

int fr_l2norm_rows_f32(const float* x, float* out, int rows, int dim, fr_stream_t stream);

size_t fr_gallery_match_workspace(int F, int64_t N);
int fr_gallery_match_f32(const float* Q, const float* G, int F, int64_t N, int D,
                         int64_t row_offset, int64_t* out_idx, float* out_score,
                         void* workspace, size_t workspace_bytes, const int32_t* seg_counts, int seg_len,
                         fr_stream_t stream);
int fr_gallery_match_view_f32(const float* Q, const float* G, const int64_t* view, int F, int64_t Nview, int D,
                              int64_t* out_idx, float* out_score, void* workspace, size_t workspace_bytes,
                              fr_stream_t stream);
int fr_gallery_update_rows_f32(float* G, const int64_t* slots, const float* rows, int n, int D, int normalise,
                               fr_stream_t stream);
#define FR_TOPK 4
#define FR_TOPK8 8
#define FR_F8_SCALE 256.0f
size_t fr_gallery_match_f16_workspace(int F, int64_t N);
int fr_gallery_match_f16(const float* Q, const void* G16, const float* G32, int F, int64_t N, int D,
                         int64_t row_offset, int64_t* out_idx, float* out_score,
                         void* workspace, size_t workspace_bytes, const int32_t* seg_counts, int seg_len,
                         fr_stream_t stream);
size_t fr_gallery_match_f8_workspace(int F, int64_t N);
int fr_gallery_match_f8(const float* Q, const void* G8, const float* G32, int F, int64_t N, int D,
                        int64_t row_offset, int64_t* out_idx, float* out_score,
                        void* workspace, size_t workspace_bytes, const int32_t* seg_counts, int seg_len,
                        fr_stream_t stream);
#define FR_TOPK_MAX 16
size_t fr_gallery_topk_workspace(int F, int64_t N, int K);
int fr_gallery_topk_f32(const float* Q, const float* G, int F, int64_t N, int D, int K, int64_t row_offset,
                        int64_t* out_idx , float* out_score , void* workspace,
                        size_t workspace_bytes, const int32_t* seg_counts, int seg_len, fr_stream_t stream);
int fr_gallery_topk_view_f32(const float* Q, const float* G, const int64_t* view, int F, int64_t Nview, int D,
                             int K, int64_t* out_idx, float* out_score, void* workspace,
                             size_t workspace_bytes, fr_stream_t stream);
#define FR_SHADOW_F16 1
#define FR_SHADOW_F8 2
int fr_gallery_update_rows_shadow(float* G, void* shadow, int shadow_kind, const int64_t* slots, const float* rows,
                                  int n, int D, int normalise, fr_stream_t stream);
size_t fr_gallery_match_view_f16_workspace(int F, int64_t Nview);
int fr_gallery_match_view_f16(const float* Q, const void* S16, const float* G32, const int64_t* view, int F,
                              int64_t Nview, int64_t capacity, int D, int64_t* out_idx, float* out_score,
                              void* workspace, size_t workspace_bytes, fr_stream_t stream);
size_t fr_gallery_match_view_f8_workspace(int F, int64_t Nview);
int fr_gallery_match_view_f8(const float* Q, const void* S8, const float* G32, const int64_t* view, int F,
                             int64_t Nview, int64_t capacity, int D, int64_t* out_idx, float* out_score,
                             void* workspace, size_t workspace_bytes, fr_stream_t stream);
size_t fr_gallery_topk_f16_workspace(int F, int64_t N, int K);
int fr_gallery_topk_f16(const float* Q, const void* G16, const float* G32, int F, int64_t N, int D, int K,
                        int64_t row_offset, const float* gmax, int64_t* out_idx, float* out_score, int32_t* flags,
                        void* workspace, size_t workspace_bytes, const int32_t* seg_counts, int seg_len,
                        fr_stream_t stream);
size_t fr_gallery_topk_view_f16_workspace(int F, int64_t Nview, int K);
int fr_gallery_topk_view_f16(const float* Q, const void* S16, const float* G32, const int64_t* view, int F,
                             int64_t Nview, int64_t capacity, int D, int K, const float* gmax, int64_t* out_idx,
                             float* out_score, int32_t* flags, void* workspace, size_t workspace_bytes,
                             fr_stream_t stream);
int fr_gallery_topk_view_masked_f32(const float* Q, const float* G, const int64_t* view, int F, int64_t Nview, int D,
                                    int K, int64_t* out_idx, float* out_score, void* workspace,
                                    size_t workspace_bytes, const int32_t* mask, fr_stream_t stream);
int fr_gallery_gmax_update(const float* G, const int64_t* slots, int64_t n, int D, float* gmax, fr_stream_t stream);
size_t fr_gallery_match_grouped_workspace(int ngroups, int64_t max_view_len);
int fr_gallery_match_grouped_f32(const float* Q, const float* G, const int64_t* views, const int64_t* gtab,
                                 const int32_t* qmap, int F, int ngroups, int64_t max_view_len, int64_t capacity, int D,
                                 int64_t* out_idx, float* out_score, void* workspace, size_t workspace_bytes,
                                 const int32_t* seg_counts, int seg_len, fr_stream_t stream);
size_t fr_gallery_topk_grouped_workspace(int ngroups, int64_t max_view_len, int K);
int fr_gallery_topk_grouped_f32(const float* Q, const float* G, const int64_t* views, const int64_t* gtab,
                                const int32_t* qmap, int F, int ngroups, int64_t max_view_len, int64_t capacity, int D,
                                int K, int64_t* out_idx , float* out_score , void* workspace,
                                size_t workspace_bytes, const int32_t* seg_counts, int seg_len, fr_stream_t stream);
int fr_f32_to_f8(const float* x, void* out, int64_t n, fr_stream_t stream);
int fr_f32_to_f16(const float* x, void* out, int64_t n, fr_stream_t stream);
int fr_match_decide(const int64_t* idx, const float* score, int F, float thr, float unknown_thr,
                    int32_t* decision, fr_stream_t stream);


int fr_match_pack_candidates(const int64_t* idx, const float* score, int n, int32_t* cand, fr_stream_t stream);
int fr_match_reduce_shards(const int32_t* cand_all, int R, int n, int q0, int F, int64_t* out_idx,
                           float* out_score, fr_stream_t stream);
int fr_match_reduce_shards_topk(const int32_t* cand_all, int R, int n, int K, int q0, int F,
                                int64_t* out_idx, float* out_score, fr_stream_t stream);
int fr_exchange_pack_queries(const float* Q, int F, int q_max, int D, float* send, fr_stream_t stream);
int fr_exchange_counts(const float* gathered, int R, int q_max, int D, int32_t* counts, fr_stream_t stream);


int fr_gallery_first_above_f32(const float* Q, const float* G, int F, int64_t N, int D, float thr,
                               int inclusive, int64_t row_offset, int64_t* out_idx, float* out_score,
                               void* workspace, size_t workspace_bytes, fr_stream_t stream);
int fr_cosine_matrix_f32(const float* A, const float* B, int F, int N, int D, float* out,
                         fr_stream_t stream);
int fr_mean_rows_f32(const float* x, int K, int D, float* out, fr_stream_t stream);
#define FR_UNKNOWN_N 0
#define FR_UNKNOWN_OVERFLOW 1
#define FR_UNKNOWN_HEADER 4
#define FR_UNKNOWN_STATE_INTS(capacity) (FR_UNKNOWN_HEADER + 3 * (capacity))
int fr_unknown_assign_batch_f32(const float* E, const int32_t* take, int F, int D, float thr, float* avg, float* hist,
                                int32_t* state, int capacity, int depth, int32_t* out_cluster, int32_t* out_new,
                                int32_t* out_count, fr_stream_t stream);

int fr_gallery_first_above_blocked_f32(const float* Q, const float* G, const int64_t* view, const int32_t* take, int F,
                                       int64_t N, int D, float thr, int inclusive, int64_t row_offset, int64_t* out_idx,
                                       float* out_score, void* workspace, size_t workspace_bytes, fr_stream_t stream);
#define FR_ENROL_DONE 0
#define FR_ENROL_NO_FACE 1
#define FR_ENROL_DIFFERENT 2
#define FR_ENROL_DUPLICATE 3
#define FR_ENROL_MAX_POSES 8
#define FR_ENROL_MAX_JOBS 256
size_t fr_enrol_batch_workspace(int J, int64_t N);
int fr_enrol_batch_f32(const float* E, const float* bbox, int S, const int32_t* img_first, const int32_t* img_count, int I,
                       const int32_t* job_first, int J, int max_poses, int D, const float* G, const int64_t* view, int64_t N,
                       float sim_thr, float dup_thr, int32_t* status, int32_t* pair, int32_t* face, float* avg, float* row,
                       int64_t* dup_pos, float* dup_score, void* workspace, size_t workspace_bytes, fr_stream_t stream);
#define FR_PAIRS_OVERFLOW 1
#define FR_PAIRS_NONFINITE 2
size_t fr_gallery_pairs_workspace(int64_t N, int64_t capacity);
int fr_gallery_pairs_above_f16(const float* G32, const int64_t* view, int64_t N, int D, float thr, int inclusive,
                               int64_t capacity, int max_ranges, int64_t* out_key, float* out_score, int32_t* out_counts,
                               void* workspace, size_t workspace_bytes, fr_stream_t stream);

typedef struct {
    const void* x; const void* w; void* y;
    const float* bias; const float* slope; const void* residual;
    float* out_f32_partial;
    int B, H, W, Cin, Cout, KH, KW, stride, pad, Ho, Wo;
    int bias_mode; int splitk;
    const void* x2; int C2;
} fr_conv_args;
int fr_conv_nhwc_f16(const fr_conv_args* args, fr_stream_t stream);
typedef struct {
    const void* x8; const void* w8; void* y16; void* y8;
    const float* oscale; const float* bias; const float* slope; const void* residual;
    int B, H, W, Cin, Cout, bias_mode;
    float y8_mul;
    const float* y8_sub;
} fr_conv_f8_args;
int fr_conv_nhwc_f8(const fr_conv_f8_args* args, fr_stream_t stream);
int fr_quantize_f16_f8(const void* x16, void* out8, int64_t n, float mul, fr_stream_t stream);
int fr_quantize_f16_f8_centred(const void* x16, void* out8, int64_t n, int C, const float* sub, float mul,
                               fr_stream_t stream);
size_t fr_conv_stage14_weight_bytes(int nconv);
int fr_conv_stage14_pack(const void* w, void* out, fr_stream_t stream);
int fr_conv_stage14_f16(const void* x, void* y, const void* wstream, const float* params, int B, int nblocks,
                        fr_stream_t stream);
size_t fr_conv_stage28_weight_bytes(int nconv);
int fr_conv_stage28_pack(const void* w, void* out, fr_stream_t stream);
int fr_conv_stage28_f16(void* x, void* mid, const void* wstream, const float* params, int B, int nblocks, fr_stream_t stream);
size_t fr_conv_walk64_weight_bytes(int Cout);
int fr_conv_walk64_pack(const void* w, void* out, int Cout, fr_stream_t stream);
int fr_conv_walk64_f16(const void* x, const void* wstream, void* y, const float* bias, int bias_mode, const float* slope,
                       const void* residual, int B, int HW, int Cout, fr_stream_t stream);
size_t fr_conv_stage14_f8_weight_bytes(int nconv);
size_t fr_conv_stage14_f8_param_floats(void);
int fr_conv_stage14_f8_pack(const void* w8, void* out, fr_stream_t stream);
int fr_conv_stage14_f8(const void* x8, const void* x16, void* y16, const void* wstream, const float* params, int B,
                       int nblocks, fr_stream_t stream);
int fr_gptq_round_e4m3(const double* W, const double* U, const float* sw, float* Q, int rows, int K, fr_stream_t stream);
int fr_conv_splitk_epilogue(const float* partial, int splitk, int M, int Cout, int Ho, int Wo,
                            const float* bias, int bias_mode, const float* slope, const void* residual,
                            void* y, fr_stream_t stream);
int fr_conv_inblock_f16(const fr_conv_args* args, fr_stream_t stream);
typedef struct {
    int kind;
    fr_conv_args args;
} fr_conv_step;
int fr_conv_sequence(const fr_conv_step* steps, int nsteps, fr_stream_t stream);
int fr_fc_reduce_l2norm(const float* partial, int splitk, int B, int dim, const float* bias,
                        float* embedding, float* normed, fr_stream_t stream);


int fr_warp_affine_5pt(const uint8_t* frames, int nframes, int H, int W, const float* kps,
                       const int32_t* frame_idx, const int32_t* count, int F, int size,
                       void* out_f16_nhwc8, uint8_t* out_u8_bgr, float* M_out, fr_stream_t stream);

int fr_warp_affine_5pt_slots(const uint8_t* frames, int nframes, int H, int W, const float* kps,
                             const int32_t* counts, int cap, int size, void* out_f16_nhwc8,
                             fr_stream_t stream);

typedef struct {
    const uint8_t* data;
    int32_t H, W, nh, nw;
    int32_t reserved[2];
} fr_frame_ref;
int fr_warp_affine_5pt_refs(const fr_frame_ref* refs, int nframes, const float* kps, const int32_t* frame_idx,
                            const int32_t* count, int F, int size, void* out_f16_nhwc8, uint8_t* out_u8_bgr,
                            float* M_out, fr_stream_t stream);
int fr_warp_affine_5pt_slots_refs(const fr_frame_ref* refs, int nframes, const float* kps, const int32_t* counts,
                                  int cap, int size, void* out_f16_nhwc8, fr_stream_t stream);

int fr_pyramid_resize_norm(const uint8_t* frames, int nframes, int H, int W, int hs, int ws,
                           float* out, fr_stream_t stream);
int fr_dconv_f32(const float* x, const float* w, const float* bias, const float* slope, float* y,
                 int B, int H, int W, int Cin, int Cout, int CoutP, int KH, int KW, int pool2,
                 const float* head_w, const float* head_b, int nhead, fr_stream_t stream);
int fr_dconv_mfma_f32(int layer, const float* x, const float* w, const float* bias, const float* slope,
                      float* y, int B, int H, int W, const float* head_w, const float* head_b,
                      const uint8_t* frames, int FH, int FW, const int32_t* counts, int cap, void* y_split,
                      fr_stream_t stream);
int fr_crop_conv1_f32(int net, const uint8_t* frames, int nframes, int H, int W, const float* boxes,
                      const int32_t* counts, int cap, const float* w, const float* bias, const float* slope,
                      float* y, fr_stream_t stream);
int fr_crop_conv1_split(int net, const uint8_t* frames, int nframes, int H, int W, const float* boxes,
                        const int32_t* counts, int cap, const float* w, const float* bias, const float* slope,
                        void* y_split, int conv_f16, fr_stream_t stream);
int fr_crop_conv1_list_f32(int net, const uint8_t* frames, int nframes, int H, int W, const float* boxes, int cap,
                           const int32_t* list, const int32_t* list_count, int list_cap, const float* w,
                           const float* bias, const float* slope, float* y, fr_stream_t stream);
int fr_ro_conv2_split(int net, const void* x_split, const float* w, const float* bias, const float* slope, float* y,
                      int nslots, const int32_t* counts, int cap, int32_t* zero_word, fr_stream_t stream);
size_t fr_ro_gemm_weight_bytes(int layer);
int fr_ro_gemm_pack(int layer, const float* w, void* out, fr_stream_t stream);
int fr_ro_gemm_split(int layer, const float* x, const void* w_packed, const float* bias, const float* slope, float* y,
                     int nslots, const int32_t* counts, int cap, fr_stream_t stream);
int fr_ro_margin_list(const float* head, int nhead, const int32_t* counts, int nframes, int cap, float logit_thr,
                      float margin, int32_t* list, int32_t* list_count, int list_cap, fr_stream_t stream);
int fr_ro_scatter_rows(const float* src, const int32_t* list, const int32_t* list_count, int list_cap, int ncols,
                       float* dst, fr_stream_t stream);
size_t fr_pnet23_workspace_bytes(int B, int H1, int W1);
int fr_pnet23_split_f16(const float* x1, const void* x1s, int B, int H1, int W1, const float* w2, const float* b2, const float* s2,
                        const float* w3, const float* b3, const float* s3, const float* hw, const float* hb,
                        float* head, int all_heads, float refine_logit_thr, float refine_band_hi, int32_t* refined_count,
                        void* workspace, size_t workspace_bytes, fr_stream_t stream);
int fr_maxpool_f32(const float* x, float* y, int B, int H, int W, int C, int k, int stride,
                   fr_stream_t stream);
int fr_pnet_candidates(const float* head, int nframes, int hc, int wc, float scale, float thr, int cap,
                       float* boxes, float* scores, float* regs, int32_t* counts,
                       int32_t* block_counts, float* prob_out, const float* dl, float dl_min, fr_stream_t stream);
int fr_sort_nms(const float* boxes, const float* scores, const float* aux, int naux,
                const int32_t* counts, int L, int nseg, int seg_cap, int seg_major, float thr, int mode,
                int max_keep,
                float* boxes_out, float* scores_out, float* aux_out, int32_t* counts_out,
                int cap_out, fr_stream_t stream);
int fr_box_refine(float* boxes, const float* aux, int naux, const int32_t* counts, int L, int cap,
                  int mode, fr_stream_t stream);
int fr_crop_resize_norm(const uint8_t* frames, int nframes, int H, int W, const float* boxes,
                        const int32_t* counts, int cap, int size, float* out, fr_stream_t stream);
int fr_stage_select(const float* boxes, const float* head, int nh, const int32_t* counts, int L, int cap,
                    float thr, float* boxes_out, float* scores_out, float* aux_out, int naux,
                    int32_t* counts_out, float* prob_out, fr_stream_t stream);

int fr_pnet_conv1_band(int mode, const uint8_t* frames, int B, int FH, int FW, int H, int W, const float* w, const float* bias,
                       const float* slope, float* y, void* y_split, const int32_t* list, const int32_t* list_count, int list_cap,
                       fr_stream_t stream);
size_t fr_pnet_band_tiles_count(int B, int H1, int W1);
int fr_pnet_band_tiles(const void* workspace, int B, int H1, int W1, int32_t* tbuf, int32_t* tiles, fr_stream_t stream);
typedef struct {
    const float* x1; float* head; void* workspace;
    int H1, W1; float scale;
    float* boxes; float* scores; float* regs; int32_t* counts; int32_t* block_counts;
    void* x1s;
    int hs, ws;
    int f16;
} fr_pnet_level;
int fr_pnet_finish_levels(const fr_pnet_level* levels, int nlevels, int nframes, const float* w2, const float* b2,
                          const float* s2, const float* w3, const float* b3, const float* s3, const float* hw,
                          const float* hb, float thr, int cap, float dl_min, int32_t* refined_count, fr_stream_t stream);
int fr_pnet_pyramid_conv1(int mode, const uint8_t* frames, int B, int FH, int FW, const fr_pnet_level* levels, int nlevels,
                          const float* w, const float* bias, const float* slope, const int32_t* list, const int32_t* list_count,
                          int list_cap, fr_stream_t stream);
int fr_pnet_pyramid_p23(const fr_pnet_level* levels, int nlevels, int nframes, const float* w2, const float* b2, const float* s2,
                        const float* w3, const float* b3, const float* s3, const float* hw, const float* hb, int all_heads,
                        float refine_logit_thr, float refine_band_hi, fr_stream_t stream);
int fr_pnet_pyramid_band_tiles(const fr_pnet_level* levels, int nlevels, int nframes, int32_t* tbuf, int32_t* tiles, fr_stream_t stream);

int fr_letterbox_u8(const fr_frame_ref* refs, int nframes, uint8_t* canvas, int dh, int dw, fr_stream_t stream);
int fr_detections_unscale(float* boxes, float* kps, const int32_t* counts, const float* det_scale, int nframes, int cap,
                          fr_stream_t stream);

#define FR_YUV_NV12 0
#define FR_YUV_I420 1
int fr_yuv420_to_bgr_u8(const uint8_t* src, uint8_t* dst, int N, int H, int W, int layout, int y_off, int cy, int cub, int cug,
                        int cvg, int cvr, fr_stream_t stream);
int fr_yuv420_to_bgr_refs_u8(const fr_frame_ref* dst_refs, const uint8_t* const* src_ptrs, int nframes, int layout, int y_off,
                             int cy, int cub, int cug, int cvg, int cvr, fr_stream_t stream);

int fr_frame_activity_u8(const uint8_t* frames, int N, int H, int W, const int32_t* slot, int S, uint8_t* grid, int32_t* geom,
                         int32_t* idle, int C, uint8_t* cur, int32_t* changed, int32_t* active, int thr, int min_cells,
                         int max_idle, fr_stream_t stream);
int fr_frame_activity_refs_u8(const fr_frame_ref* refs, int nframes, const int32_t* slot, int S, uint8_t* grid, int32_t* geom,
                              int32_t* idle, int C, uint8_t* cur, int32_t* changed, int32_t* active, int thr, int min_cells,
                              int max_idle, fr_stream_t stream);

size_t fr_det_conv_weight_halves(int Cin, int cout_packed, int K);
int fr_det_conv_f16(const void* x, const void* w, const float* bias, const void* residual, void* y, int N, int H, int W,
                    int Cin, int cout_packed, int K, int stride, int pad, int Ho, int Wo, int cout_store, int ldo,
                    int relu, int out_f32, int tile, fr_stream_t stream);
int fr_det_conv_act_f16(const void* x, const void* w, const float* bias, const float* slope, const void* residual, void* y,
                        int N, int H, int W, int Cin, int cout_packed, int K, int stride, int pad, int Ho, int Wo,
                        int cout_store, int ldo, int act, int out_f32, int tile, fr_stream_t stream);
int fr_dw_conv_f16(const void* x, const void* w, const float* bias, const float* slope, void* y, int N, int H, int W, int C, int K,
                   int stride, int pad, int Ho, int Wo, int act, fr_stream_t stream);
int fr_det_input_f16(const uint8_t* canvas, void* y, int N, int H, int W, fr_stream_t stream);
int fr_det_pool_f16(const void* x, void* y, int N, int H, int W, int C, int Ho, int Wo, int kind, int k, int stride,
                    int pad, fr_stream_t stream);
int fr_det_upsample_add_f16(const void* coarse, const void* lateral, void* y, int N, int H, int W, int C, int up,
                            fr_stream_t stream);
int fr_scrfd_decode(const float* score, const float* bbox, const float* kps, int nframes, int Hl, int Wl, int A, int stride,
                    int level, float logit_thr, const float* det_scale, int cap, float* boxes, float* scores, float* aux,
                    int32_t* counts, fr_stream_t stream);

enum { FR_FN_DCONV_MFMA = 1, FR_FN_PNET23 = 2, FR_FN_PNET_CANDIDATES = 3, FR_FN_SORT_NMS = 4, FR_FN_BOX_REFINE = 5,
       FR_FN_CROP_CONV1 = 6, FR_FN_STAGE_SELECT = 7,
       FR_FN_EVENT_RECORD = 8 , FR_FN_STREAM_WAIT = 9  };
typedef struct {
    int32_t fn; int32_t nargs;
    uint64_t a[22];
} fr_call;
int fr_detect_sequence(const fr_call* calls, int ncalls);

#ifdef __cplusplus
}
#endif
#endif
```

Baseline: 25490.

## Add coarse single-plane f16 PNet conv2/3 pass with exact re-evaluation of candidates

Adds a coarse PNet conv2/conv3/head kernel that uses only the high f16 plane, needing one MFMA per step where the split-precision path uses three. Cells whose coarse logit passes a lowered threshold (by a configurable margin) go into a list, and a second kernel re-evaluates only those cells with the full split-precision path. This cuts matrix work and LDS footprint across the whole pyramid. In exchange it adds an extra kernel, gathers per candidate, and a risk of missed detections if the margin is too small. The path is gated by coarse_p23 and band mode.

```diff
diff --git a/facerecognition_infrenceengine_amd/_lib.py b/facerecognition_infrenceengine_amd/_lib.py
--- a/facerecognition_infrenceengine_amd/_lib.py
+++ b/facerecognition_infrenceengine_amd/_lib.py
@@ -159,6 +159,9 @@
     "fr_pnet_conv1_band": (_I, [_I, _P, _I, _I, _I, _I, _I, _P, _P, _P, _P, _P, _P, _P, _I, _P]),
     "fr_pnet_band_tiles_count": (_Z, [_I, _I, _I]),
     "fr_pnet_band_tiles": (_I, [_P, _I, _I, _I, _P, _P, _P]),
+    "fr_pnet23_coarse_workspace_bytes": (_Z, [_I, _I, _I]),
+    "fr_pnet23_coarse_f16": (_I, [_P, _P, _I, _I, _I, _P, _P, _P, _P, _P, _P, _P, _P, _P, _I, _F, _F, _P, _P, _Z, _F, _P, _Z, _P, _P]),
+    "fr_pnet_pyramid_p23_coarse": (_I, [C.POINTER(PnetLevel), _I, _I, _P, _P, _P, _P, _P, _P, _P, _P, _I, _F, _F, _F, C.POINTER(_P), _P, _P]),
     "fr_pnet_finish_levels": (_I, [C.POINTER(PnetLevel), _I, _I, _P, _P, _P, _P, _P, _P, _P, _P, _F, _I, _F, _P, _P]),
     "fr_pnet_pyramid_conv1": (_I, [_I, _P, _I, _I, _I, C.POINTER(PnetLevel), _I, _P, _P, _P, _P, _P, _I, _P]),
     "fr_pnet_pyramid_p23": (_I, [C.POINTER(PnetLevel), _I, _I, _P, _P, _P, _P, _P, _P, _P, _P, _I, _F, _F, _P]),
diff --git a/facerecognition_infrenceengine_amd/csrc/pnet_fused.hip b/facerecognition_infrenceengine_amd/csrc/pnet_fused.hip
--- a/facerecognition_infrenceengine_amd/csrc/pnet_fused.hip
+++ b/facerecognition_infrenceengine_amd/csrc/pnet_fused.hip
@@ -25,20 +25,16 @@
     float logit_thr;
     float band_hi;
     int B, H1, W1, H3, W3, tiles_x, tiles_y, ntiles;
+    int* clist; int* ccounts;
+    float coarse_thr;
+    int* visited;
 };
 
-__device__ __forceinline__ void pnet23_body(const P23Args& a, const int vb, const int vgrid, char* lds) {
-#if defined(__HIP_DEVICE_COMPILE__)
-    char* x1t = lds;
-    char* x2t = x1t + 2 * P23_X1PL;
-    char* wf = x2t + 2 * P23_X2PL;
-    float* cst = reinterpret_cast<float*>(wf + 30 * 1024);
-    int* lcnt = reinterpret_cast<int*>(cst + 104);
-    const int tid = threadIdx.x, lane = tid & 63, wave = tid >> 6;
-    const int fr = lane & 15, fq = lane >> 4;
-
-    for (int e = tid; e < 30 * 64; e += P23_NT) {
-        const int l2 = e & 63, plane = (e >> 6) & 1, slot = e >> 7;
+template <int NP, int NT>
+__device__ __forceinline__ void p23_stage_weights(const P23Args& a, char* wf, float* cst) {
+    const int tid = threadIdx.x;
+    for (int e = tid; e < 15 * NP * 64; e += NT) {
+        const int l2 = e & 63, plane = NP == 2 ? (e >> 6) & 1 : 0, slot = e / (64 * NP);
         const int r = l2 & 15, q = l2 >> 4;
         const bool c3 = slot >= 5;
         const int ct = c3 ? (slot - 5) / 5 : 0, ks = c3 ? (slot - 5) % 5 : slot;
@@ -48,11 +44,26 @@
         for (int j = 0; j < 8; ++j) o[j] = split_f16_plane(w[j], plane);
         *reinterpret_cast<half8*>(wf + (size_t)e * 16) = o;
     }
-    for (int e = tid; e < 16; e += P23_NT) { cst[e] = a.b2[e]; cst[16 + e] = a.s2[e] - 1.f; }
-    for (int e = tid; e < 32; e += P23_NT) { cst[32 + e] = a.b3[e]; cst[64 + e] = a.s3[e] - 1.f; }
-    for (int e = tid; e < 8; e += P23_NT) cst[96 + e] = e < 6 ? a.hb[e] : 0.f;
+    for (int e = tid; e < 16; e += NT) { cst[e] = a.b2[e]; cst[16 + e] = a.s2[e] - 1.f; }
+    for (int e = tid; e < 32; e += NT) { cst[32 + e] = a.b3[e]; cst[64 + e] = a.s3[e] - 1.f; }
+    for (int e = tid; e < 8; e += NT) cst[96 + e] = e < 6 ? a.hb[e] : 0.f;
+}
+
+template <bool COARSE>
+__device__ __forceinline__ void pnet23_body(const P23Args& a, const int vb, const int vgrid, char* lds) {
+#if defined(__HIP_DEVICE_COMPILE__)
+    constexpr int NP = COARSE ? 1 : 2;
+    char* x1t = lds;
+    char* x2t = x1t + NP * P23_X1PL;
+    char* wf = x2t + NP * P23_X2PL;
+    float* cst = reinterpret_cast<float*>(wf + NP * 15 * 1024);
+    int* lcnt = reinterpret_cast<int*>(cst + 104);
+    const int tid = threadIdx.x, lane = tid & 63, wave = tid >> 6;
+    const int fr = lane & 15, fq = lane >> 4;
+
+    p23_stage_weights<NP, P23_NT>(a, wf, cst);
     if (tid == 0) *lcnt = 0;
-    int* const seg = a.list + (size_t)vb * a.seg_cap;
+    int* const seg = (COARSE ? a.clist : a.list) + (size_t)vb * a.seg_cap;
 
     int off2[5], off3[5];
 #pragma unroll
@@ -64,9 +75,10 @@
     }
 
     __amdgpu_buffer_rsrc_t xrs = buffer_rsrc(a.x1s, a.x1s_bytes);
-    int wy[4], wx[4], wc[4];
-#pragma unroll
-    for (int i = 0; i < 4; ++i) {
+    constexpr int NPIECE = 14 * NP, NI = (NPIECE + 7) / 8;
+    int wy[NI], wx[NI], wc[NI];
+#pragma unroll
+    for (int i = 0; i < NI; ++i) {
         const int j = wave + 8 * i, pl = j >= 14 ? 1 : 0;
         const int p = (j - 14 * pl) * 32 + (lane >> 1);
         wy[i] = p < P23_X1PX ? p / P23_X1W : 1 << 20; wx[i] = p % P23_X1W;
@@ -77,9 +89,9 @@
         const int n = tile / per, rem = tile - n * per;
         const int ty0 = (rem / a.tiles_x) * P23_RH, tx0 = (rem % a.tiles_x) * P23_RW;
 #pragma unroll
-        for (int i = 0; i < 4; ++i) {
+        for (int i = 0; i < NI; ++i) {
             const int j = wave + 8 * i;
-            if (j < 28) {
+            if (j < NPIECE) {
                 const int gy = ty0 + wy[i], gx = tx0 + wx[i];
                 const unsigned off = (gy < a.H1 && gx < a.W1) ? (unsigned)(((n * a.H1 + gy) * a.W1 + gx) * 64 + wc[i]) : 0x80000000u;
                 __builtin_amdgcn_raw_ptr_buffer_load_lds(xrs, (lds_ptr_t)(x1t + (j >= 14 ? P23_X1PL + (j - 14) * 1024 : j * 1024)), 16, off, 0, 0, 0);
@@ -95,6 +107,7 @@
         const float w = fr < 6 ? a.hw[co * 6 + fr] : 0.f;
         split_f16(w, hwh, hwl, j);
     }
+    (void)hwl;
     issue_window(vb);
     for (int tile = vb; tile < a.ntiles; tile += vgrid) {
         const int per = a.tiles_x * a.tiles_y;
@@ -115,17 +128,27 @@
             }
 #pragma unroll
             for (int ks = 0; ks < 5; ++ks) {
-                const half8 ahi = *reinterpret_cast<const half8*>(wf + ((ks * 2 + 0) * 64 + lane) * 16);
-                const half8 alo = *reinterpret_cast<const half8*>(wf + ((ks * 2 + 1) * 64 + lane) * 16);
-#pragma unroll
-                for (int t = 0; t < 3; ++t) {
-                    if (t < nt) {
-                        const char* bp = x1t + (pb[t] + off2[ks]);
-                        const half8 bhi = *reinterpret_cast<const half8*>(bp);
-                        const half8 blo = *reinterpret_cast<const half8*>(bp + P23_X1PL);
-                        acc[t] = __builtin_amdgcn_mfma_f32_16x16x32_f16(alo, bhi, acc[t], 0, 0, 0);
-                        acc[t] = __builtin_amdgcn_mfma_f32_16x16x32_f16(ahi, blo, acc[t], 0, 0, 0);
-                        acc[t] = __builtin_amdgcn_mfma_f32_16x16x32_f16(ahi, bhi, acc[t], 0, 0, 0);
+                const half8 ahi = *reinterpret_cast<const half8*>(wf + ((ks * NP + 0) * 64 + lane) * 16);
+                if constexpr (COARSE) {
+#pragma unroll
+                    for (int t = 0; t < 3; ++t) {
+                        if (t < nt) {
+                            const half8 bhi = *reinterpret_cast<const half8*>(x1t + (pb[t] + off2[ks]));
+                            acc[t] = __builtin_amdgcn_mfma_f32_16x16x32_f16(ahi, bhi, acc[t], 0, 0, 0);
+                        }
+                    }
+                } else {
+                    const half8 alo = *reinterpret_cast<const half8*>(wf + ((ks * 2 + 1) * 64 + lane) * 16);
+#pragma unroll
+                    for (int t = 0; t < 3; ++t) {
+                        if (t < nt) {
+                            const char* bp = x1t + (pb[t] + off2[ks]);
+                            const half8 bhi = *reinterpret_cast<const half8*>(bp);
+                            const half8 blo = *reinterpret_cast<const half8*>(bp + P23_X1PL);
+                            acc[t] = __builtin_amdgcn_mfma_f32_16x16x32_f16(alo, bhi, acc[t], 0, 0, 0);
+                            acc[t] = __builtin_amdgcn_mfma_f32_16x16x32_f16(ahi, blo, acc[t], 0, 0, 0);
+                            acc[t] = __builtin_amdgcn_mfma_f32_16x16x32_f16(ahi, bhi, acc[t], 0, 0, 0);
+                        }
                     }
                 }
             }
@@ -137,12 +160,19 @@
                     float4v v = acc[t] + bb;
 #pragma unroll
                     for (int e = 0; e < 4; ++e) v[e] = __builtin_fmaf(fminf(v[e], 0.f), ss[e], v[e]);
-                    half4 hi, lo;
-#pragma unroll
-                    for (int e = 0; e < 4; ++e) split_f16(v[e], hi, lo, e);
                     char* o = x2t + q * 32 + fq * 8;
-                    *reinterpret_cast<half4*>(o) = hi;
-                    *reinterpret_cast<half4*>(o + P23_X2PL) = lo;
+                    if constexpr (COARSE) {
+                        half4 hi;
+#pragma unroll
+                        for (int e = 0; e < 4; ++e) hi[e] = (half_t)v[e];
+                        *reinterpret_cast<half4*>(o) = hi;
+                    } else {
+                        half4 hi, lo;
+#pragma unroll
+                        for (int e = 0; e < 4; ++e) split_f16(v[e], hi, lo, e);
+                        *reinterpret_cast<half4*>(o) = hi;
+                        *reinterpret_cast<half4*>(o + P23_X2PL) = lo;
+                    }
                 }
             }
         }
@@ -159,6 +189,18 @@
             }
 #pragma unroll
             for (int ks = 0; ks < 5; ++ks) {
+                if constexpr (COARSE) {
+                    half8 ahi[2];
+#pragma unroll
+                    for (int ct = 0; ct < 2; ++ct) ahi[ct] = *reinterpret_cast<const half8*>(wf + ((5 + ct * 5 + ks) * 64 + lane) * 16);
+#pragma unroll
+                    for (int t = 0; t < 2; ++t) {
+                        const half8 bhi = *reinterpret_cast<const half8*>(x2t + (pb[t] + off3[ks]));
+#pragma unroll
+                        for (int ct = 0; ct < 2; ++ct) acc[t][ct] = __builtin_amdgcn_mfma_f32_16x16x32_f16(ahi[ct], bhi, acc[t][ct], 0, 0, 0);
+                    }
+                    continue;
+                }
                 half8 ahi[2], alo[2];
 #pragma unroll
                 for (int ct = 0; ct < 2; ++ct) {
@@ -192,8 +234,10 @@
                     bh[4 + e] = h1; bl[4 + e] = (half_t)(x1 - (float)h1);
                 }
                 float4v d = {0.f, 0.f, 0.f, 0.f};
-                d = __builtin_amdgcn_mfma_f32_16x16x32_f16(hwl, bh, d, 0, 0, 0);
-                d = __builtin_amdgcn_mfma_f32_16x16x32_f16(hwh, bl, d, 0, 0, 0);
+                if constexpr (!COARSE) {
+                    d = __builtin_amdgcn_mfma_f32_16x16x32_f16(hwl, bh, d, 0, 0, 0);
+                    d = __builtin_amdgcn_mfma_f32_16x16x32_f16(hwh, bl, d, 0, 0, 0);
+                }
                 d = __builtin_amdgcn_mfma_f32_16x16x32_f16(hwh, bh, d, 0, 0, 0);
                 const int q = (wave * 2 + t) * 16 + fr;
                 const int gy = ty0 + (q >> 5), gx = tx0 + (q & 31);
@@ -203,7 +247,7 @@
                 const float o0 = d[0] + hb4[0], o1 = d[1] + hb4[1];
                 const float dlv = __shfl(o1 - o0, fr, 64);
                 const bool band = a.band_hi > a.logit_thr;
-                const bool flag = inb && fq == 0 && (split_nonfinite(dlv) || (dlv >= a.logit_thr && (!band || dlv <= a.band_hi)));
+                const bool flag = inb && fq == 0 && (split_nonfinite(dlv) || (COARSE ? dlv >= a.coarse_thr : (dlv >= a.logit_thr && (!band || dlv <= a.band_hi))));
                 const unsigned long long fm = __ballot(flag);
                 if (fm) {
                     int base = 0;
@@ -213,7 +257,7 @@
                 }
                 if (inb) {
                     if (fq == 0) a.dl[cell] = o1 - o0;
-                    if (a.all_heads || (band && dlv >= a.logit_thr)) {
+                    if (!COARSE && (a.all_heads || (band && dlv >= a.logit_thr))) {
                         float* o = a.head + cell * 6 + 4 * fq;
                         *reinterpret_cast<float2*>(o) = make_float2(o0, o1);
                         if (fq == 0) *reinterpret_cast<float2*>(o + 2) = make_float2(d[2] + hb4[2], d[3] + hb4[3]);
@@ -223,13 +267,17 @@
         }
     }
     __syncthreads();
-    if (tid == 0) a.counts[vb] = *lcnt;
+    if (tid == 0) (COARSE ? a.ccounts : a.counts)[vb] = *lcnt;
 #endif
 }
 
 __global__ __launch_bounds__(P23_NT, 4) void pnet23_split_f16(P23Args a) {
     extern __shared__ __attribute__((aligned(16))) char lds[];
-    pnet23_body(a, (int)blockIdx.x, (int)gridDim.x, lds);
+    pnet23_body<false>(a, (int)blockIdx.x, (int)gridDim.x, lds);
+}
+__global__ __launch_bounds__(P23_NT, 4) void pnet23_coarse_f16(P23Args a) {
+    extern __shared__ __attribute__((aligned(16))) char lds[];
+    pnet23_body<true>(a, (int)blockIdx.x, (int)gridDim.x, lds);
 }
 
 #define P23_MAXL 16
@@ -248,7 +296,182 @@
     a.x1s = t.x1s[l]; a.x1s_bytes = (unsigned)a.B * a.H1 * a.W1 * 64; a.head = t.head[l];
     a.dl = t.dl[l]; a.counts = reinterpret_cast<int*>(a.dl + (size_t)a.B * a.H3 * a.W3); a.list = a.counts + 512;
     a.seg_cap = t.seg_cap[l];
-    pnet23_body(a, (int)blockIdx.x - t.first[l], t.first[l + 1] - t.first[l], lds);
+    pnet23_body<false>(a, (int)blockIdx.x - t.first[l], t.first[l + 1] - t.first[l], lds);
+}
+
+struct P23Coarse { int* buf[P23_MAXL]; };
+__device__ __forceinline__ int p23_find_level(const P23Levels& t, const int g) {
+    int l = 0;
+    while (l + 1 < t.nlevels && g >= t.first[l + 1]) ++l;
+    return l;
+}
+__device__ __forceinline__ void p23_set_level(P23Args& a, const P23Levels& t, const P23Coarse& c, const int l) {
+    a.H1 = t.H1[l]; a.W1 = t.W1[l]; a.H3 = a.H1 - 4; a.W3 = a.W1 - 4;
+    a.tiles_x = (a.W3 + P23_RW - 1) / P23_RW; a.tiles_y = (a.H3 + P23_RH - 1) / P23_RH;
+    a.ntiles = a.B * a.tiles_x * a.tiles_y;
+    a.x1s = t.x1s[l]; a.x1s_bytes = (unsigned)a.B * a.H1 * a.W1 * 64; a.head = t.head[l];
+    a.dl = t.dl[l]; a.counts = reinterpret_cast<int*>(a.dl + (size_t)a.B * a.H3 * a.W3); a.list = a.counts + 512;
+    a.seg_cap = t.seg_cap[l];
+    a.ccounts = c.buf[l]; a.clist = c.buf[l] + 512;
+}
+__global__ __launch_bounds__(P23_NT, 4) void pnet23_coarse_levels(P23Args a, P23Levels t, P23Coarse c) {
+    extern __shared__ __attribute__((aligned(16))) char lds[];
+    const int l = p23_find_level(t, (int)blockIdx.x);
+    p23_set_level(a, t, c, l);
+    pnet23_body<true>(a, (int)blockIdx.x - t.first[l], t.first[l + 1] - t.first[l], lds);
+}
+
+#define P23R_NT 256
+#define P23R_SLOT 1616
+#define P23R_LO 800
+#define P23R_LDS ((size_t)30 * 1024 + 108 * 4 + (P23R_NT / 64) * 16 * P23R_SLOT)
+__global__ __launch_bounds__(P23R_NT, 1) void pnet23_reeval_levels(P23Args a, P23Levels t, P23Coarse c) {
+#if defined(__HIP_DEVICE_COMPILE__)
+    extern __shared__ __attribute__((aligned(16))) char lds[];
+    char* wf = lds;
+    float* cst = reinterpret_cast<float*>(wf + 30 * 1024);
+    const int tid = threadIdx.x, lane = tid & 63, wave = tid >> 6;
+    const int fr = lane & 15, fq = lane >> 4;
+    char* const win = reinterpret_cast<char*>(cst + 108) + wave * (16 * P23R_SLOT);
+    p23_stage_weights<2, P23R_NT>(a, wf, cst);
+    half8 hwh, hwl;
+#pragma unroll
+    for (int j = 0; j < 8; ++j) {
+        const int co = j < 4 ? 4 * fq + j : 16 + 4 * fq + (j - 4);
+        const float w = fr < 6 ? a.hw[co * 6 + fr] : 0.f;
+        split_f16(w, hwh, hwl, j);
+    }
+    __syncthreads();
+    const float4v bb = *reinterpret_cast<const float4v*>(cst + 4 * fq), ss = *reinterpret_cast<const float4v*>(cst + 16 + 4 * fq);
+    const float4v b30 = *reinterpret_cast<const float4v*>(cst + 32 + 4 * fq), s30 = *reinterpret_cast<const float4v*>(cst + 64 + 4 * fq);
+    const float4v b31 = *reinterpret_cast<const float4v*>(cst + 48 + 4 * fq), s31 = *reinterpret_cast<const float4v*>(cst + 80 + 4 * fq);
+    const float4v hb4 = *reinterpret_cast<const float4v*>(cst + 96 + 4 * (fq & 1));
+    const bool band = a.band_hi > a.logit_thr;
+    char* const xc = win + fr * P23R_SLOT + (fq & 1) * 16;
+    int pj[25], psrc[25], pdst[25];
+    const int nseg = t.first[t.nlevels];
+    for (int g = (int)blockIdx.x * (P23R_NT / 64) + wave; g < nseg; g += (int)gridDim.x * (P23R_NT / 64)) {
+        const int l = p23_find_level(t, g);
+        p23_set_level(a, t, c, l);
+        const int vb = g - t.first[l];
+        const int n_list = a.ccounts[vb];
+        const int* const lst = a.clist + (size_t)vb * a.seg_cap;
+        int* const seg = a.list + (size_t)vb * a.seg_cap;
+        const int hw3 = a.H3 * a.W3;
+        int nflag = 0;
+        if (a.visited && lane == 0 && n_list) atomicAdd(a.visited, n_list);
+#pragma unroll
+        for (int it = 0; it < 25; ++it) {
+            const int idx = it * 64 + lane, j = idx / 100, rem = idx - j * 100, px = rem >> 2, ch = rem & 3;
+            pj[it] = j;
+            psrc[it] = ((px / 5) * a.W1 + px % 5) * 64 + ch * 16;
+            pdst[it] = j * P23R_SLOT + (ch >> 1) * P23R_LO + px * 32 + (ch & 1) * 16;
+        }
+        auto corner_of = [&](int i0) {
+            const int cell = lst[min(i0 + fr, n_list - 1)];
+            const int n = cell / hw3, rem = cell - n * hw3, y = rem / a.W3, x = rem - y * a.W3;
+            return ((n * a.H1 + y) * a.W1 + x) * 64;
+        };
+        float4v pf[25];
+        if (n_list > 0) {
+            const int corner = corner_of(0);
+#pragma unroll
+            for (int it = 0; it < 25; ++it)
+                pf[it] = *reinterpret_cast<const float4v*>(a.x1s + (size_t)(unsigned)(__shfl(corner, pj[it], 64) + psrc[it]));
+        }
+        for (int i0 = 0; i0 < n_list; i0 += 16) {
+            const int cell = lst[min(i0 + fr, n_list - 1)];
+#pragma unroll
+            for (int it = 0; it < 25; ++it) *reinterpret_cast<float4v*>(win + pdst[it]) = pf[it];
+            __builtin_amdgcn_wave_barrier();
+            if (i0 + 16 < n_list) {
+                const int corner = corner_of(i0 + 16);
+#pragma unroll
+                for (int it = 0; it < 25; ++it)
+                    pf[it] = *reinterpret_cast<const float4v*>(a.x1s + (size_t)(unsigned)(__shfl(corner, pj[it], 64) + psrc[it]));
+            }
+            float4v acc2[9];
+#pragma unroll
+            for (int p = 0; p < 9; ++p) acc2[p] = float4v{0.f, 0.f, 0.f, 0.f};
+#pragma unroll
+            for (int ks = 0; ks < 5; ++ks) {
+                int tp = 2 * ks + (fq >> 1);
+                if (tp > 8) tp = 8;
+                const half8 ahi = *reinterpret_cast<const half8*>(wf + ((ks * 2 + 0) * 64 + lane) * 16);
+                const half8 alo = *reinterpret_cast<const half8*>(wf + ((ks * 2 + 1) * 64 + lane) * 16);
+#pragma unroll
+                for (int p = 0; p < 9; ++p) {
+                    const char* bp = xc + ((p / 3 + tp / 3) * 5 + (p % 3 + tp % 3)) * 32;
+                    const half8 bhi = *reinterpret_cast<const half8*>(bp);
+                    const half8 blo = *reinterpret_cast<const half8*>(bp + P23R_LO);
+                    acc2[p] = __builtin_amdgcn_mfma_f32_16x16x32_f16(alo, bhi, acc2[p], 0, 0, 0);
+                    acc2[p] = __builtin_amdgcn_mfma_f32_16x16x32_f16(ahi, blo, acc2[p], 0, 0, 0);
+                    acc2[p] = __builtin_amdgcn_mfma_f32_16x16x32_f16(ahi, bhi, acc2[p], 0, 0, 0);
+                }
+            }
+            __builtin_amdgcn_wave_barrier();
+#pragma unroll
+            for (int p = 0; p < 9; ++p) {
+                float4v v = acc2[p] + bb;
+#pragma unroll
+                for (int e = 0; e < 4; ++e) v[e] = __builtin_fmaf(fminf(v[e], 0.f), ss[e], v[e]);
+                half4 hi, lo;
+#pragma unroll
+                for (int e = 0; e < 4; ++e) split_f16(v[e], hi, lo, e);
+                char* o = win + fr * P23R_SLOT + p * 32 + fq * 8;
+                *reinterpret_cast<half4*>(o) = hi;
+                *reinterpret_cast<half4*>(o + P23R_LO) = lo;
+            }
+            __builtin_amdgcn_wave_barrier();
+            float4v acc3[2] = {float4v{0.f, 0.f, 0.f, 0.f}, float4v{0.f, 0.f, 0.f, 0.f}};
+#pragma unroll
+            for (int ks = 0; ks < 5; ++ks) {
+                int tp = 2 * ks + (fq >> 1);
+                if (tp > 8) tp = 8;
+                const half8 bhi = *reinterpret_cast<const half8*>(xc + tp * 32);
+                const half8 blo = *reinterpret_cast<const half8*>(xc + tp * 32 + P23R_LO);
+#pragma unroll
+                for (int ct = 0; ct < 2; ++ct) {
+                    const half8 ahi = *reinterpret_cast<const half8*>(wf + (((5 + ct * 5 + ks) * 2 + 0) * 64 + lane) * 16);
+                    const half8 alo = *reinterpret_cast<const half8*>(wf + (((5 + ct * 5 + ks) * 2 + 1) * 64 + lane) * 16);
+                    acc3[ct] = __builtin_amdgcn_mfma_f32_16x16x32_f16(alo, bhi, acc3[ct], 0, 0, 0);
+                    acc3[ct] = __builtin_amdgcn_mfma_f32_16x16x32_f16(ahi, blo, acc3[ct], 0, 0, 0);
+                    acc3[ct] = __builtin_amdgcn_mfma_f32_16x16x32_f16(ahi, bhi, acc3[ct], 0, 0, 0);
+                }
+            }
+            __builtin_amdgcn_wave_barrier();
+            const float4v v0 = acc3[0] + b30, v1 = acc3[1] + b31;
+            half8 bh, bl;
+#pragma unroll
+            for (int e = 0; e < 4; ++e) {
+                const float x0 = __builtin_fmaf(fminf(v0[e], 0.f), s30[e], v0[e]), x1 = __builtin_fmaf(fminf(v1[e], 0.f), s31[e], v1[e]);
+                const half_t h0 = (half_t)x0, h1 = (half_t)x1;
+                bh[e] = h0; bl[e] = (half_t)(x0 - (float)h0);
+                bh[4 + e] = h1; bl[4 + e] = (half_t)(x1 - (float)h1);
+            }
+            float4v d = {0.f, 0.f, 0.f, 0.f};
+            d = __builtin_amdgcn_mfma_f32_16x16x32_f16(hwl, bh, d, 0, 0, 0);
+            d = __builtin_amdgcn_mfma_f32_16x16x32_f16(hwh, bl, d, 0, 0, 0);
+            d = __builtin_amdgcn_mfma_f32_16x16x32_f16(hwh, bh, d, 0, 0, 0);
+            const bool inb = fq < 2 && i0 + fr < n_list;
+            const float o0 = d[0] + hb4[0], o1 = d[1] + hb4[1];
+            const float dlv = __shfl(o1 - o0, fr, 64);
+            const bool flag = inb && fq == 0 && (split_nonfinite(dlv) || (dlv >= a.logit_thr && (!band || dlv <= a.band_hi)));
+            const unsigned long long fm = __ballot(flag);
+            if (flag) seg[nflag + (int)__builtin_popcountll(fm & ((1ull << lane) - 1ull))] = cell;
+            nflag += (int)__builtin_popcountll(fm);
+            if (inb) {
+                if (fq == 0) a.dl[cell] = o1 - o0;
+                if (band && dlv >= a.logit_thr) {
+                    float* o = a.head + (size_t)cell * 6 + 4 * fq;
+                    *reinterpret_cast<float2*>(o) = make_float2(o0, o1);
+                    if (fq == 0) *reinterpret_cast<float2*>(o + 2) = make_float2(d[2] + hb4[2], d[3] + hb4[3]);
+                }
+            }
+        }
+        if (lane == 0) a.counts[vb] = nflag;
+    }
+#endif
 }
 
 #define PREF_WS 304
@@ -400,22 +623,63 @@
     return (size_t)ncell * 4 + 512 * 4 + (size_t)grid * seg_cap * 4;
 }
 
+extern "C" size_t fr_pnet23_coarse_workspace_bytes(int B, int H1, int W1) {
+    if (B <= 0 || H1 < 5 || W1 < 5) return 0;
+    long long ncell, ntiles; int grid, seg_cap;
+    p23_layout(B, H1, W1, ncell, ntiles, grid, seg_cap);
+    return 512 * 4 + (size_t)grid * seg_cap * 4;
+}
+
+static unsigned p23_reeval_grid(long long segments) {
+    const long long blocks = (segments + P23R_NT / 64 - 1) / (P23R_NT / 64);
+    return (unsigned)(blocks < 256 ? blocks : 256);
+}
+
+constexpr size_t P23_LDS = (size_t)2 * P23_X1PL + (size_t)2 * P23_X2PL + 30 * 1024 + 108 * 4;
+constexpr size_t P23C_LDS = (size_t)P23_X1PL + (size_t)P23_X2PL + 15 * 1024 + 108 * 4;
+
+static int p23_level(const char* who, const float* x1, const void* x1s, int B, int H1, int W1, const float* w2, const float* b2,
+                     const float* s2, const float* w3, const float* b3, const float* s3, const float* hw,
+                     const float* hb, float* head, int all_heads, float refine_logit_thr, float refine_band_hi,
+                     int32_t* refined_count, void* workspace, size_t workspace_bytes, float coarse_margin, void* coarse,
+                     size_t coarse_bytes, int32_t* visited_count, fr_stream_t stream);
+
 extern "C" int fr_pnet23_split_f16(const float* x1, const void* x1s, int B, int H1, int W1, const float* w2, const float* b2,
                                    const float* s2, const float* w3, const float* b3, const float* s3, const float* hw,
                                    const float* hb, float* head, int all_heads, float refine_logit_thr, float refine_band_hi,
                                    int32_t* refined_count, void* workspace, size_t workspace_bytes, fr_stream_t stream) {
-    FR_REQUIRE(x1 && x1s && w2 && b2 && s2 && w3 && b3 && s3 && hw && hb && head, "fr_pnet23_split_f16: null pointer");
-    FR_REQUIRE((int64_t)B * H1 * W1 * 64 < (1ll << 31), "fr_pnet23_split_f16: the split conv1 map must stay below 2 GiB (got %lld bytes)", (long long)B * H1 * W1 * 64);
-    FR_REQUIRE(B > 0 && H1 >= 5 && W1 >= 5, "fr_pnet23_split_f16: the conv1 map must be at least 5x5 (got %dx%d)", H1, W1);
+    return p23_level("fr_pnet23_split_f16", x1, x1s, B, H1, W1, w2, b2, s2, w3, b3, s3, hw, hb, head, all_heads, refine_logit_thr,
+                     refine_band_hi, refined_count, workspace, workspace_bytes, 0.f, nullptr, 0, nullptr, stream);
+}
+
+extern "C" int fr_pnet23_coarse_f16(const float* x1, const void* x1s, int B, int H1, int W1, const float* w2, const float* b2,
+                                    const float* s2, const float* w3, const float* b3, const float* s3, const float* hw,
+                                    const float* hb, float* head, int all_heads, float refine_logit_thr, float refine_band_hi,
+                                    int32_t* refined_count, void* workspace, size_t workspace_bytes, float coarse_margin,
+                                    void* coarse, size_t coarse_bytes, int32_t* visited_count, fr_stream_t stream) {
+    FR_REQUIRE(!(all_heads & 1), "fr_pnet23_coarse_f16: all_heads & 1 (the approximate heads of every cell) needs fr_pnet23_split_f16");
+    FR_REQUIRE(coarse && coarse_margin >= 0.f, "fr_pnet23_coarse_f16: needs a coarse buffer and a margin >= 0");
+    return p23_level("fr_pnet23_coarse_f16", x1, x1s, B, H1, W1, w2, b2, s2, w3, b3, s3, hw, hb, head, all_heads, refine_logit_thr,
+                     refine_band_hi, refined_count, workspace, workspace_bytes, coarse_margin, coarse, coarse_bytes, visited_count, stream);
+}
+
+static int p23_level(const char* who, const float* x1, const void* x1s, int B, int H1, int W1, const float* w2, const float* b2,
+                     const float* s2, const float* w3, const float* b3, const float* s3, const float* hw,
+                     const float* hb, float* head, int all_heads, float refine_logit_thr, float refine_band_hi,
+                     int32_t* refined_count, void* workspace, size_t workspace_bytes, float coarse_margin, void* coarse,
+                     size_t coarse_bytes, int32_t* visited_count, fr_stream_t stream) {
+    FR_REQUIRE(x1 && x1s && w2 && b2 && s2 && w3 && b3 && s3 && hw && hb && head, "%s: null pointer", who);
+    FR_REQUIRE((int64_t)B * H1 * W1 * 64 < (1ll << 31), "%s: the split conv1 map must stay below 2 GiB (got %lld bytes)", who, (long long)B * H1 * W1 * 64);
+    FR_REQUIRE(B > 0 && H1 >= 5 && W1 >= 5, "%s: the conv1 map must be at least 5x5 (got %dx%d)", who, H1, W1);
     P23Args a;
     a.x1 = x1; a.x1s = (const unsigned char*)x1s; a.x1s_bytes = (unsigned)((int64_t)B * H1 * W1 * 64); a.w2 = w2; a.b2 = b2; a.s2 = s2; a.w3 = w3; a.b3 = b3; a.s3 = s3; a.hw = hw; a.hb = hb; a.head = head; a.all_heads = all_heads & 1;
     a.B = B; a.H1 = H1; a.W1 = W1; a.H3 = H1 - 4; a.W3 = W1 - 4;
     a.tiles_x = (a.W3 + P23_RW - 1) / P23_RW; a.tiles_y = (a.H3 + P23_RH - 1) / P23_RH;
     long long ncell, nt; int grid, seg_cap;
     p23_layout(B, H1, W1, ncell, nt, grid, seg_cap);
-    FR_REQUIRE(nt < (1ll << 31) && ncell < (1ll << 31), "fr_pnet23_split_f16: too many tiles");
+    FR_REQUIRE(nt < (1ll << 31) && ncell < (1ll << 31), "%s: too many tiles", who);
     const size_t need = fr_pnet23_workspace_bytes(B, H1, W1);
-    FR_REQUIRE(workspace && workspace_bytes >= need, "fr_pnet23_split_f16: workspace needs %zu bytes (fr_pnet23_workspace_bytes)", need);
+    FR_REQUIRE(workspace && workspace_bytes >= need, "%s: workspace needs %zu bytes (fr_pnet23_workspace_bytes)", who, need);
     a.dl = reinterpret_cast<float*>(workspace);
     a.counts = reinterpret_cast<int*>(a.dl + ncell);
     a.list = a.counts + 512;
@@ -423,12 +687,30 @@
     a.logit_thr = refine_logit_thr;
     a.band_hi = refine_band_hi;
     a.ntiles = (int)nt;
-    constexpr size_t lds = (size_t)2 * P23_X1PL + (size_t)2 * P23_X2PL + 30 * 1024 + 108 * 4;
-    static FrDevLatch latch;
-    if (!fr_raise_lds(reinterpret_cast<const void*>(pnet23_split_f16), lds, latch)) { fr_set_error("fr_pnet23_split_f16: cannot raise dynamic LDS"); return FR_E_LAUNCH; }
+    a.clist = a.ccounts = a.visited = nullptr; a.coarse_thr = 0.f;
     hipStream_t s = fr_stream(stream);
-    pnet23_split_f16<<<grid, P23_NT, lds, s>>>(a);
-    FR_CHECK_LAUNCH("pnet23_split_f16");
+    if (coarse) {
+        const size_t cneed = fr_pnet23_coarse_workspace_bytes(B, H1, W1);
+        FR_REQUIRE(coarse_bytes >= cneed, "%s: the coarse buffer needs %zu bytes (fr_pnet23_coarse_workspace_bytes)", who, cneed);
+        a.ccounts = reinterpret_cast<int*>(coarse); a.clist = a.ccounts + 512;
+        a.coarse_thr = refine_logit_thr - coarse_margin; a.visited = visited_count;
+        static FrDevLatch latch0, latch1;
+        if (!fr_raise_lds(reinterpret_cast<const void*>(pnet23_coarse_f16), P23C_LDS, latch0) ||
+            !fr_raise_lds(reinterpret_cast<const void*>(pnet23_reeval_levels), P23R_LDS, latch1)) { fr_set_error("fr_pnet23_coarse_f16: cannot raise dynamic LDS"); return FR_E_LAUNCH; }
+        pnet23_coarse_f16<<<grid, P23_NT, P23C_LDS, s>>>(a);
+        FR_CHECK_LAUNCH("pnet23_coarse_f16");
+        P23Levels t{};
+        P23Coarse c{};
+        t.nlevels = 1; t.x1s[0] = a.x1s; t.head[0] = head; t.dl[0] = a.dl; t.H1[0] = H1; t.W1[0] = W1; t.seg_cap[0] = seg_cap;
+        t.first[0] = 0; t.first[1] = grid; c.buf[0] = a.ccounts;
+        pnet23_reeval_levels<<<p23_reeval_grid(grid), P23R_NT, P23R_LDS, s>>>(a, t, c);
+        FR_CHECK_LAUNCH("pnet23_reeval_levels");
+    } else {
+        static FrDevLatch latch;
+        if (!fr_raise_lds(reinterpret_cast<const void*>(pnet23_split_f16), P23_LDS, latch)) { fr_set_error("fr_pnet23_split_f16: cannot raise dynamic LDS"); return FR_E_LAUNCH; }
+        pnet23_split_f16<<<grid, P23_NT, P23_LDS, s>>>(a);
+        FR_CHECK_LAUNCH("pnet23_split_f16");
+    }
     if (all_heads & 2) return FR_OK;
     PRefArgs r;
     r.x1 = x1; r.w2 = w2; r.b2 = b2; r.s2 = s2; r.w3 = w3; r.b3 = b3; r.s3 = s3; r.hw = hw; r.hb = hb; r.head = head;
@@ -513,18 +795,46 @@
     return FR_OK;
 }
 
+static int p23_pyramid(const char* who, const fr_pnet_level* levels, int nlevels, int nframes, const float* w2, const float* b2,
+                       const float* s2, const float* w3, const float* b3, const float* s3, const float* hw,
+                       const float* hb, int all_heads, float refine_logit_thr, float refine_band_hi, float coarse_margin,
+                       void* const* coarse, int32_t* visited_count, fr_stream_t stream);
+
 extern "C" int fr_pnet_pyramid_p23(const fr_pnet_level* levels, int nlevels, int nframes, const float* w2, const float* b2,
                                    const float* s2, const float* w3, const float* b3, const float* s3, const float* hw,
                                    const float* hb, int all_heads, float refine_logit_thr, float refine_band_hi, fr_stream_t stream) {
-    FR_REQUIRE(levels && nlevels > 0 && nlevels <= P23_MAXL && nframes > 0, "fr_pnet_pyramid_p23: 1 .. %d levels", P23_MAXL);
-    FR_REQUIRE(w2 && b2 && s2 && w3 && b3 && s3 && hw && hb, "fr_pnet_pyramid_p23: null pointer");
+    return p23_pyramid("fr_pnet_pyramid_p23", levels, nlevels, nframes, w2, b2, s2, w3, b3, s3, hw, hb, all_heads, refine_logit_thr,
+                       refine_band_hi, 0.f, nullptr, nullptr, stream);
+}
+
+extern "C" int fr_pnet_pyramid_p23_coarse(const fr_pnet_level* levels, int nlevels, int nframes, const float* w2, const float* b2,
+                                          const float* s2, const float* w3, const float* b3, const float* s3, const float* hw,
+                                          const float* hb, int all_heads, float refine_logit_thr, float refine_band_hi,
+                                          float coarse_margin, void* const* coarse, int32_t* visited_count, fr_stream_t stream) {
+    FR_REQUIRE(!(all_heads & 1), "fr_pnet_pyramid_p23_coarse: all_heads & 1 (the approximate heads of every cell) needs fr_pnet_pyramid_p23");
+    FR_REQUIRE(coarse && coarse_margin >= 0.f, "fr_pnet_pyramid_p23_coarse: needs the coarse buffers and a margin >= 0");
+    return p23_pyramid("fr_pnet_pyramid_p23_coarse", levels, nlevels, nframes, w2, b2, s2, w3, b3, s3, hw, hb, all_heads, refine_logit_thr,
+                       refine_band_hi, coarse_margin, coarse, visited_count, stream);
+}
+
+static int p23_pyramid(const char* who, const fr_pnet_level* levels, int nlevels, int nframes, const float* w2, const float* b2,
+                       const float* s2, const float* w3, const float* b3, const float* s3, const float* hw,
+                       const float* hb, int all_heads, float refine_logit_thr, float refine_band_hi, float coarse_margin,
+                       void* const* coarse, int32_t* visited_count, fr_stream_t stream) {
+    FR_REQUIRE(levels && nlevels > 0 && nlevels <= P23_MAXL && nframes > 0, "%s: 1 .. %d levels", who, P23_MAXL);
+    FR_REQUIRE(w2 && b2 && s2 && w3 && b3 && s3 && hw && hb, "%s: null pointer", who);
     P23Levels t;
+    P23Coarse c{};
     t.nlevels = nlevels;
     long long total = 0;
     for (int l = 0; l < nlevels; ++l) {
         const fr_pnet_level& L = levels[l];
-        FR_REQUIRE(L.x1s && L.head && L.workspace && L.H1 >= 5 && L.W1 >= 5, "fr_pnet_pyramid_p23: level %d: bad entry", l);
-        FR_REQUIRE((int64_t)nframes * L.H1 * L.W1 * 64 < (1ll << 31), "fr_pnet_pyramid_p23: level %d: the split conv1 map must stay below 2 GiB", l);
+        if (coarse) {
+            FR_REQUIRE(coarse[l], "%s: level %d: no coarse buffer", who, l);
+            c.buf[l] = reinterpret_cast<int*>(coarse[l]);
+        }
+        FR_REQUIRE(L.x1s && L.head && L.workspace && L.H1 >= 5 && L.W1 >= 5, "%s: level %d: bad entry", who, l);
+        FR_REQUIRE((int64_t)nframes * L.H1 * L.W1 * 64 < (1ll << 31), "%s: level %d: the split conv1 map must stay below 2 GiB", who, l);
         long long ncell, nt; int grid, seg_cap;
         p23_layout(nframes, L.H1, L.W1, ncell, nt, grid, seg_cap);
         t.x1s[l] = reinterpret_cast<const unsigned char*>(L.x1s); t.head[l] = L.head; t.dl[l] = reinterpret_cast<float*>(L.workspace);
@@ -536,10 +846,20 @@
     P23Args a{};
     a.w2 = w2; a.b2 = b2; a.s2 = s2; a.w3 = w3; a.b3 = b3; a.s3 = s3; a.hw = hw; a.hb = hb; a.all_heads = all_heads & 1;
     a.logit_thr = refine_logit_thr; a.band_hi = refine_band_hi; a.B = nframes;
-    constexpr size_t lds = (size_t)2 * P23_X1PL + (size_t)2 * P23_X2PL + 30 * 1024 + 108 * 4;
+    if (coarse) {
+        a.coarse_thr = refine_logit_thr - coarse_margin; a.visited = visited_count;
+        static FrDevLatch latch0, latch1;
+        if (!fr_raise_lds(reinterpret_cast<const void*>(pnet23_coarse_levels), P23C_LDS, latch0) ||
+            !fr_raise_lds(reinterpret_cast<const void*>(pnet23_reeval_levels), P23R_LDS, latch1)) { fr_set_error("fr_pnet_pyramid_p23_coarse: cannot raise dynamic LDS"); return FR_E_LAUNCH; }
+        pnet23_coarse_levels<<<(unsigned)total, P23_NT, P23C_LDS, fr_stream(stream)>>>(a, t, c);
+        FR_CHECK_LAUNCH("pnet23_coarse_levels");
+        pnet23_reeval_levels<<<p23_reeval_grid(total), P23R_NT, P23R_LDS, fr_stream(stream)>>>(a, t, c);
+        FR_CHECK_LAUNCH("pnet23_reeval_levels");
+        return FR_OK;
+    }
     static FrDevLatch latch;
-    if (!fr_raise_lds(reinterpret_cast<const void*>(pnet23_split_levels), lds, latch)) { fr_set_error("fr_pnet_pyramid_p23: cannot raise dynamic LDS"); return FR_E_LAUNCH; }
-    pnet23_split_levels<<<(unsigned)total, P23_NT, lds, fr_stream(stream)>>>(a, t);
+    if (!fr_raise_lds(reinterpret_cast<const void*>(pnet23_split_levels), P23_LDS, latch)) { fr_set_error("fr_pnet_pyramid_p23: cannot raise dynamic LDS"); return FR_E_LAUNCH; }
+    pnet23_split_levels<<<(unsigned)total, P23_NT, P23_LDS, fr_stream(stream)>>>(a, t);
     FR_CHECK_LAUNCH("pnet23_split_levels");
     return FR_OK;
 }
diff --git a/facerecognition_infrenceengine_amd/mtcnn.py b/facerecognition_infrenceengine_amd/mtcnn.py
--- a/facerecognition_infrenceengine_amd/mtcnn.py
+++ b/facerecognition_infrenceengine_amd/mtcnn.py
@@ -121,6 +121,9 @@
     use_sequence = True
     fused_crop = True
     split_ro = True
+    coarse_p23 = True
+    coarse_margin = 0.05
+    visited_cells = None
 
     def __init__(self, minsize=20, factor=0.709, fused_pnet=True, batch_min_pixels=None):
         self.minsize, self.factor = minsize, factor
@@ -144,6 +147,7 @@
     cache: bool
     recorder: bool
     split: bool
+    coarse: float
     chunks: tuple
 
 
@@ -170,7 +174,8 @@
 
 
 _PLAN_READS = ("minsize", "factor", "fused_pnet", "batch_min_pixels", "solo_max_frames", "pnet_band", "split_pconv1", "split_pconv1_min_px",
-               "pyramid_launch", "one_stream", "level_streams", "single_frame_level_streams", "split_ro", "fused_crop", "use_sequence")
+               "pyramid_launch", "one_stream", "level_streams", "single_frame_level_streams", "split_ro", "fused_crop", "use_sequence",
+               "coarse_p23", "coarse_margin")
 
 
 @functools.lru_cache(maxsize=256)
@@ -197,7 +202,8 @@
     cache = bool(eager and few and not trace and not out and not capturing)
     recorder = bool(cache and recordable and cfg.use_sequence and cfg.fused_pnet and cfg.fused_crop and not cfg.one_stream)
     split = bool(cfg.split_ro and cfg.fused_crop and batch and not trace)
-    return DetectPlan(N, scales, geo, batch, few, band, fused, f16, pyramid, eager or pyramid, nside, cache, recorder, split, chunks)
+    coarse = float(cfg.coarse_margin) if cfg.coarse_p23 and band else 0.0
+    return DetectPlan(N, scales, geo, batch, few, band, fused, f16, pyramid, eager or pyramid, nside, cache, recorder, split, coarse, chunks)
 
 
 _RO = (SimpleNamespace(name="rnet", cap_in="cap_p", cap_out="cap_r", crop=24, map1=(11, 28), map2=(4, 48), w1="_rc1", w2="_rc2",
@@ -348,12 +354,16 @@
         lt = math.log(self.thresholds[0] / (1.0 - self.thresholds[0]))
         return lt - self.refine_margin, lt + self.refine_margin if band else float("-inf")
 
-    def _level_buffers(self, N, scale, geo, band, f16, cand):
+    def _coarse(self, margin):
+        return 0.0 if self.p23_all_heads else margin
+
+    def _level_buffers(self, N, scale, geo, band, f16, cand, coarse=0.0):
         hs, ws, h, w = geo
         path = getattr(self._tls, "path", None)
         if path is not None:
             path["fused_levels"] += 1
             path["band_levels"] += int(band)
+            path["coarse_levels"] += int(coarse > 0.0)
             if f16:
                 path["pconv1_mfma_levels"].append((h, w))
         xs = self._new((N, h, w, 64), torch.uint8)
@@ -361,13 +371,14 @@
         head = self._f32(N, h - 4, w - 4, 6)
         wsp = self._new((self.lib.fr_pnet23_workspace_bytes(N, h, w) // 4,), torch.float32)
         bc = self._i32(N * (-(-(h - 4) * (w - 4) // 256)))
+        cws = self._i32(self.lib.fr_pnet23_coarse_workspace_bytes(N, h, w) // 4) if coarse > 0.0 else None
         entry = None
         if cand is not None:
             entry = _lib.PnetLevel(x.data_ptr(), head.data_ptr(), wsp.data_ptr(), h, w, float(scale), *[t.data_ptr() for t in cand],
                                    bc.data_ptr(), xs.data_ptr(), hs, ws, int(f16))
-        return dict(h=h, w=w, f16=f16, x=x, xs=xs, head=head, wsp=wsp, bc=bc), entry
-
-    def _level(self, frames, scale, geo, fused, band, f16, trace, cand):
+        return dict(h=h, w=w, f16=f16, x=x, xs=xs, head=head, wsp=wsp, bc=bc, cws=cws), entry
+
+    def _level(self, frames, scale, geo, fused, band, f16, trace, cand, coarse=0.0):
         N, H, W, _ = frames.shape
         hs, ws, h, w = geo
         lib, p1 = self.lib, self.p1
@@ -383,16 +394,22 @@
             head, h, w = self._dconv(x, self.p3, N, h, w)
             return head, h, w, self._i32(N * (-(-h * w // 256))), None, 0.0, None
         lo, hi = self._band_logits(band)
-        t, entry = self._level_buffers(N, scale, geo, band, f16, cand[3:] if f16 else None)
-        x, xs, head, wsp = t["x"], t["xs"], t["head"], t["wsp"]
+        coarse = self._coarse(coarse)
+        t, entry = self._level_buffers(N, scale, geo, band, f16, cand[3:] if f16 else None, coarse)
+        x, xs, head, wsp, cws = t["x"], t["xs"], t["head"], t["wsp"], t["cws"]
         p1w, p23 = (_lib.ptr(p1.w), _lib.ptr(p1.b), _lib.ptr(p1.slope)), [_lib.ptr(v) for v in self._p23]
         if f16:
             lib.fr_pnet_conv1_band(0, self._fptr(frames), N, H, W, hs, ws, *p1w, None, _lib.ptr(xs), None, None, 0, self._s)
         else:
             self._dconv(None, p1, N, hs, ws, frames=frames, y_split=xs, y=x)
-        lib.fr_pnet23_split_f16(_lib.ptr(x), _lib.ptr(xs), N, h, w, *p23, _lib.ptr(head),
-                                (1 if (self.p23_all_heads or trace is not None) else 0) | (2 if f16 else 0), lo, hi,
-                                _lib.ptr(self.refined_cells), _lib.ptr(wsp), wsp.numel() * 4, self._s)
+        if coarse > 0.0:
+            lib.fr_pnet23_coarse_f16(_lib.ptr(x), _lib.ptr(xs), N, h, w, *p23, _lib.ptr(head), 2 if f16 else 0, lo, hi,
+                                     _lib.ptr(self.refined_cells), _lib.ptr(wsp), wsp.numel() * 4, coarse, _lib.ptr(cws), cws.numel() * 4,
+                                     _lib.ptr(self.visited_cells), self._s)
+        else:
+            lib.fr_pnet23_split_f16(_lib.ptr(x), _lib.ptr(xs), N, h, w, *p23, _lib.ptr(head),
+                                    (1 if (self.p23_all_heads or trace is not None) else 0) | (2 if f16 else 0), lo, hi,
+                                    _lib.ptr(self.refined_cells), _lib.ptr(wsp), wsp.numel() * 4, self._s)
         keep = None
         if f16:
             nt = lib.fr_pnet_band_tiles_count(N, h, w)
@@ -412,7 +429,8 @@
         fused = bool(self.fused_pnet) and N <= _frames32(*geo[2:])
         band = bool(self.pnet_band and _is_batch(self, N, H, W) and trace is None)
         f16 = fused and cand is not None and _f16_conv1(self, band, *geo[2:])
-        head, hc, wc, _, dl, dl_min, keep = self._level(frames, scale, geo, fused, band, f16, trace, cand)
+        coarse = self.coarse_margin if self.coarse_p23 and band else 0.0
+        head, hc, wc, _, dl, dl_min, keep = self._level(frames, scale, geo, fused, band, f16, trace, cand, coarse)
         self._tls.dl, self._tls.level_done, self._tls.keep = (dl, dl_min), keep is not None, keep
         return head, hc, wc
 
@@ -421,16 +439,20 @@
         lib, p1, nlev = self.lib, self.p1, len(plan.scales)
         lo, hi = self._band_logits(plan.band)
         lv = (_lib.PnetLevel * nlev)()
-        keep, ntile, words = [], 0, 0
+        keep, ntile, words, coarse = [], 0, 0, self._coarse(plan.coarse)
         for li, (s, geo, f16) in enumerate(zip(plan.scales, plan.geo, plan.f16)):
-            t, lv[li] = self._level_buffers(N, s, geo, plan.band, f16, [c[li] for c in cand])
+            t, lv[li] = self._level_buffers(N, s, geo, plan.band, f16, [c[li] for c in cand], coarse)
             keep.append(t)
             if f16:
                 nt = lib.fr_pnet_band_tiles_count(N, t["h"], t["w"])
                 ntile, words = ntile + nt, words + (nt + 31) // 32
         p1w, p23 = (_lib.ptr(p1.w), _lib.ptr(p1.b), _lib.ptr(p1.slope)), [_lib.ptr(t) for t in self._p23]
         lib.fr_pnet_pyramid_conv1(0, self._fptr(frames), N, H, W, lv, nlev, *p1w, None, None, 0, self._s)
-        lib.fr_pnet_pyramid_p23(lv, nlev, N, *p23, 1 if self.p23_all_heads else 0, lo, hi, self._s)
+        if coarse > 0.0:
+            cws = (ctypes.c_void_p * nlev)(*[t["cws"].data_ptr() for t in keep])
+            lib.fr_pnet_pyramid_p23_coarse(lv, nlev, N, *p23, 0, lo, hi, coarse, cws, _lib.ptr(self.visited_cells), self._s)
+        else:
+            lib.fr_pnet_pyramid_p23(lv, nlev, N, *p23, 1 if self.p23_all_heads else 0, lo, hi, self._s)
         if ntile:
             tbuf, tiles = self._i32(1 + words), self._i32(ntile)
             lib.fr_pnet_pyramid_band_tiles(lv, nlev, N, _lib.ptr(tbuf), _lib.ptr(tiles), self._s)
@@ -482,7 +504,7 @@
                     lcand = [c[li] for c in cand]
                     head, hc, wc, bc, dl, dl_min, done = self._level(
                         frames, s, plan.geo[li], plan.fused[li], plan.band, plan.f16[li], trace,
-                        (float(s), t0, cs, *lcand) if plan.batch and trace is None else None)
+                        (float(s), t0, cs, *lcand) if plan.batch and trace is None else None, plan.coarse)
                     prob = self._f32(N, hc, wc) if trace is not None else None
                     if done is not None:
                         keep.append(done)
@@ -646,7 +668,7 @@
         known = key in caches
         tls.cache = [caches.setdefault(key, []), 0]
         cfg = (self.fused_pnet, self.fused_crop, self.p23_all_heads, self.thresholds, self.refine_margin,
-               self.cap_scale, self.keep_scale, self.cap_p, self.cap_r, self.cap_o, self.minsize, self.factor)
+               self.cap_scale, self.keep_scale, self.cap_p, self.cap_r, self.cap_o, self.minsize, self.factor, self.coarse_p23, self.coarse_margin)
         seq = seqs.get(key)
         if seq is not None and (not plan.recorder or seq["cfg"] != cfg):
             seqs.pop(key)
@@ -680,7 +702,7 @@
         with torch.cuda.device(self.device):
             plan = detect_plan(N, H, W, self, trace is not None, level_streams, _out is not None, torch.cuda.is_current_stream_capturing())
             if _out is None:
-                self._tls.path = {"frames": N, "batch": plan.batch, "chunks": max(1, len(plan.chunks)), "fused_levels": 0, "band_levels": 0,
+                self._tls.path = {"frames": N, "batch": plan.batch, "chunks": max(1, len(plan.chunks)), "fused_levels": 0, "band_levels": 0, "coarse_levels": 0,
                                   "pconv1_mfma_levels": [], "unfused_levels": 0, "split_ro": False, "exact_lists": []}
                 self._tls.exact_counters = []
             if plan.chunks:
diff --git a/include/frhip.h b/include/frhip.h
--- a/include/frhip.h
+++ b/include/frhip.h
@@ -239,6 +239,12 @@
                         const float* w3, const float* b3, const float* s3, const float* hw, const float* hb,
                         float* head, int all_heads, float refine_logit_thr, float refine_band_hi, int32_t* refined_count,
                         void* workspace, size_t workspace_bytes, fr_stream_t stream);
+size_t fr_pnet23_coarse_workspace_bytes(int B, int H1, int W1);
+int fr_pnet23_coarse_f16(const float* x1, const void* x1s, int B, int H1, int W1, const float* w2, const float* b2, const float* s2,
+                         const float* w3, const float* b3, const float* s3, const float* hw, const float* hb,
+                         float* head, int all_heads, float refine_logit_thr, float refine_band_hi, int32_t* refined_count,
+                         void* workspace, size_t workspace_bytes, float coarse_margin, void* coarse, size_t coarse_bytes,
+                         int32_t* visited_count, fr_stream_t stream);
 int fr_maxpool_f32(const float* x, float* y, int B, int H, int W, int C, int k, int stride,
                    fr_stream_t stream);
 int fr_pnet_candidates(const float* head, int nframes, int hc, int wc, float scale, float thr, int cap,
@@ -280,6 +286,10 @@
                         const float* w3, const float* b3, const float* s3, const float* hw, const float* hb, int all_heads,
                         float refine_logit_thr, float refine_band_hi, fr_stream_t stream);
 int fr_pnet_pyramid_band_tiles(const fr_pnet_level* levels, int nlevels, int nframes, int32_t* tbuf, int32_t* tiles, fr_stream_t stream);
+int fr_pnet_pyramid_p23_coarse(const fr_pnet_level* levels, int nlevels, int nframes, const float* w2, const float* b2, const float* s2,
+                               const float* w3, const float* b3, const float* s3, const float* hw, const float* hb, int all_heads,
+                               float refine_logit_thr, float refine_band_hi, float coarse_margin, void* const* coarse,
+                               int32_t* visited_count, fr_stream_t stream);
 
 int fr_letterbox_u8(const fr_frame_ref* refs, int nframes, uint8_t* canvas, int dh, int dw, fr_stream_t stream);
 int fr_detections_unscale(float* boxes, float* kps, const int32_t* counts, const float* det_scale, int nframes, int cap,
```

Result: faster. 26410 (median of 6 runs) (+3.6%).
